# tencent-ailab/pika

Measured on NVIDIA H100. Metric: utterances/sec RNN-T train step (T=1000,U=150,V=6k), higher is better.
Workload: dtype bf16

## Files before the change

include/pika_b200.h:

```cpp
#ifndef PIKA_B200_H
#define PIKA_B200_H
#include <stdint.h>

#ifdef __cplusplus
extern "C" {
#endif

#define PK_F32 0
#define PK_BF16 1

const char* pk_last_error(void);
int pk_version(void);
long long pk_launch_count(void);

#define PK_GEMM_MAX_PAIRS 9
#define PK_SEL_ZERO 0
#define PK_SEL_ZB0 1
#define PK_SEL_ZB1 2
#define PK_SEL_KZ 3
#define PK_ACT_NONE 0
#define PK_ACT_RELU 1
#define PK_AUX_NONE 0
#define PK_AUX_ADD 1
#define PK_AUX_MASK_NZ 2

typedef struct {
    const void* ptr;
    int64_t dim[4];
    int64_t stride[3];
} pk_view4;

typedef struct {
    int n_pairs;
    pk_view4 a[PK_GEMM_MAX_PAIRS];
    pk_view4 b[PK_GEMM_MAX_PAIRS];
    int a_row_off[PK_GEMM_MAX_PAIRS];
    int b_row_off[PK_GEMM_MAX_PAIRS];
    int a_mn_major, b_mn_major;
    int a_sel2, a_sel3, b_sel2, b_sel3;
    int kz_count;
    pk_view4 c;
    int c_dtype;
    int c_accumulate;
    float alpha;
    const float* bias;
    int act;
    float drop_p;
    uint32_t drop_seed;
    int aux_mode;
    const void* aux;
    int aux_dtype;
    int64_t aux_stride[3];
    float aux_scale;
    int block_n;
    int k_splits;
    float* row_lse;
} pk_gemm_desc;

int pk_gemm_bf16(const pk_gemm_desc* desc, void* stream);
int pk_gemm_row_lse_parts(long long M, long long N, int block_n);

long long pk_rnnt_loss_workspace_bytes(int B, int T, int U1);
long long pk_rnnt_loss_colsum_workspace_bytes(int B, int T, int U1, int ldv);
int pk_rnnt_loss_fwd_bwd(const void* logits, int dtype, const int* labels, const int* frame_lens,
                         const int* label_lens, int B, int T, int U1, int V, int ldv, int ld_labels,
                         const float* grad_scale, float* costs, void* dlogits, float* dlogits_colsum, void* workspace,
                         long long workspace_bytes, void* stream);
int pk_rnnt_loss_fwd_bwd_lse(const void* logits, int dtype, const int* labels, const int* frame_lens,
                             const int* label_lens, int B, int T, int U1, int V, int ldv, int ld_labels,
                             const float* grad_scale, float* costs, void* dlogits, float* dlogits_colsum, void* workspace,
                             long long workspace_bytes, const float* row_lse, int n_parts, void* stream);

int pk_cast_split(const void* src, int src_dtype, long long ld_src, void* hi, void* lo, long long ld_dst,
                  long long rows, int cols, int cols_pad, float scale, void* stream);
int pk_attention_lse_stride(int T);
int pk_attention_fwd(const void* q, const void* k, const void* v, long long ld_qkv, void* out, long long ld_out, float* lse,
                     int B, int T, int heads, int dh, float alpha, float drop_p, uint32_t seed, void* stream);
int pk_attention_bwd(const void* q, const void* k, const void* v, long long ld_qkv, const void* out, long long ld_out,
                     const void* dout, long long ld_dout, const float* lse, float* dsum_ws, void* dq, void* dk, void* dv,
                     long long ld_dqkv, int B, int T, int heads, int dh, float alpha, float drop_p, uint32_t seed, void* stream);
long long pk_colstats_ws_floats(int C);
int pk_bn_fwd(const void* x, void* y, int dtype, long long rows, int C, const float* w, const float* b, float eps,
              int train, float momentum, float* run_mean, float* run_var, float* mean, float* rstd, float* stats_ws,
              void* stream);
int pk_bn_bwd(const void* dy, const void* x, void* dx, int dtype, long long rows, int C, const float* w,
              const float* mean, const float* rstd, int train, int relu_mask, float* dw, float* db, float* ws ,
              void* stream);
int pk_colsum(const void* x, int dtype, long long rows, int C, float* out, float* ws, void* stream);
int pk_layernorm_fwd(const void* x, void* y, int dtype, long long rows, int C, const float* w, const float* b, float eps,
                     float* mean, float* rstd, void* stream);
int pk_layernorm_bwd(const void* dy, const void* x, void* dx, int dtype, long long rows, int C, const float* w,
                     const float* mean, const float* rstd, float* dw, float* db, void* stream);
int pk_softmax_fwd(const float* S, long long ld_s, void* P, void* Pd, int dtype, long long ld_p, long long rows, int n,
                   float drop_p, uint32_t seed, void* stream);
int pk_softmax_masked_fwd(const float* S, long long ld_s, void* P, void* Pd, int dtype, long long ld_p, long long rows, int n,
                          int q_len, int heads, int causal, const uint8_t* key_pad, float drop_p, uint32_t seed, void* stream);
int pk_softmax_bwd(const float* dPd, long long ld_d, const void* P, long long ld_p, void* dS, int dtype, long long rows,
                   int n, float drop_p, uint32_t seed, void* stream);
#define PK_RELPOS_MAX 1024
int pk_softmax_masked_relpos_fwd(const float* S, long long ld_s, const float* QR, long long ld_r, void* P, void* Pd, int dtype,
                                 long long ld_p, long long rows, int n, int q_len, int heads, int causal, const uint8_t* key_pad,
                                 int max_rel, float* Pb, float drop_p, uint32_t seed, void* stream);
int pk_softmax_relpos_bwd(const float* dPd, long long ld_d, const float* G, long long ld_r, const void* P, long long ld_p, void* dS,
                          int dtype, long long rows, int n, int q_len, int heads, int max_rel, float* dSb, float drop_p,
                          uint32_t seed, void* stream);
int pk_dropout(const void* x, void* y, int dtype, long long n, float p, uint32_t seed, void* stream);
int pk_mask_nz(const void* dy, const void* y, void* dx, int dtype, long long n, float scale, void* stream);
int pk_add(const void* a, const void* b, void* o, int dtype, long long n, void* stream);
int pk_log_softmax(const void* x, int dtype, long long ld, float* y, long long rows, int n, float scale, void* stream);
int pk_joint_gate_fwd(const void* ex, const void* py, void* h, int dtype, int B, int T, int U1, int H, int ld_h, void* stream);
int pk_joint_gate_bwd(const void* ex, const void* py, const void* dh, void* dex, void* dpy, int dtype, int B, int T, int U1,
                      int H, void* stream);
int pk_lstm_cell_fwd(const float* gx, long long ld_gx, const float* gh, long long ld_gh, const float* c_prev, float* c_out,
                     void* h_out, int dtype, long long ld_h, float* gates_save, int B, int H, void* stream);
int pk_lstm_cell_bwd(const void* dh_out, long long ld_dho, const float* dh_rec, const float* dc_next, const float* gates,
                     const float* c, const float* c_prev, void* dgates, int dtype, float* dc_prev, int B, int H, void* stream);
int pk_embedding_fwd(const long long* idx, const float* table, int E, void* out, int dtype, int ld_out, long long n, void* stream);
int pk_embedding_bwd(const long long* idx, const void* dout, int dtype, int ld, int E, float* dtable, long long n,
                     long long padding_idx, void* stream);

int pk_absmax(const float* x, long long n, float* out, int* nan_flag, void* stream);
int pk_sgd_nesterov_clip(float* p, const float* g, float* buf, long long n, float lr, float momentum, float max_norm,
                         const float* absmax, const int* nan_flag, int first, void* stream);
int pk_bmuf_delta(const float* glob, const float* local, float* delta, long long n, void* stream);
int pk_bmuf_update(float* glob, float* local, float* delta_prev, const float* delta_sum, long long n, int world,
                   float block_momentum, float block_lr, void* stream);

long long pk_frontend_workspace_bytes(int B, int n_max, int t_max, int n_mel, int D);
int pk_frontend_fwd(const short* pcm, long long ld_pcm, const int* n_samples, const float* rate, const int* new_len,
                    const float* target_db, const int* n_frames, int B, int n_max, int t_max, int n_mel, int lctx,
                    int rctx, const float* window, const float* twiddle, const float* mel_w, const int* mel_lo,
                    const int* mel_hi, float preemph, int cmn, const float* offset, const float* scale, int f0, int fs,
                    int t0, int ts, void* out, int out_dtype, short* wave_i16_out, void* workspace,
                    long long workspace_bytes, int* err_flag, float dither, unsigned int dither_seed, void* stream);
int pk_fbank(const float* wave, long long ld_wave, const int* n_frames, int B, int t_max, int n_mel, const float* window,
             const float* twiddle, const float* mel_w, const int* mel_lo, const int* mel_hi, float preemph, float* feats,
             float dither, unsigned int dither_seed, void* stream);

int pk_beam_prepare(const int* next_ys, const int* step_ctx, int* t_idx, const void* enc, int dtype, int Tenc, int H, void* enc_hid,
                    const float* embed, int E, void* x_emb, int ld_x, int K, int blk, int rows, void* stream);
int pk_beam_lstm_cell(const float* gates, const int* next_ys, const int* step_ctx, int blk, void* h, int dtype, float* c, int rows, int H,
                      void* stream);
int pk_beam_step_end(int* step_ctx, const int* not_done, int max_steps, void* stream);
int pk_beam_gate(const float* a, void* h, int dtype, int rows, int H, void* stream);
int pk_row_lse(const void* x, int dtype, long long ld, float* lse, long long rows, int n, float scale, void* stream);
int pk_beam_advance(const float* logits, int ldv, const float* row_lse, float sm_scale, const int* t_idx, const int* num_frames, const int* max_len, float* scores,
                    int* next_ys, int* prev_ks, int* hyp_tok, int* hyp_len, float* fin_score, int* fin_step, int* fin_k,
                    int* fin_count, int* eos_top, int* done, int* not_done_total, int B, int K, int V, int L, int cap,
                    const int* step_ctx, int blk, int n_best, int beam_prune, void* stream);
int pk_beam_reorder(const int* prev_ks, const int* step_ctx, const void* h_in, const float* c_in, const int* t_in, void* h_out, float* c_out,
                    int* t_out, int dtype, int K, int H, int layers, int rows, void* stream);
typedef struct {
    const int* arc_off;
    const int* arc_ilabel;
    const double* arc_weight;
    const int* arc_next;
    const double* finals;
    int backoff_id, n_disambig;
    int disambig_ids[4];
} pk_lm_fst;
int pk_beam_advance_lm(const float* logits, int ldv, const float* row_lse, float sm_scale, const int* t_idx, const int* num_frames, const int* max_len, float* scores,
                       int* next_ys, int* prev_ks, int* hyp_tok, int* hyp_len, float* fin_score, int* fin_step, int* fin_k,
                       int* fin_count, int* eos_top, int* done, int* not_done_total, int B, int K, int V, int L, int cap,
                       const int* step_ctx, int blk, int n_best, int beam_prune, const pk_lm_fst* fst, double lm_scale, double nonblk_reward,
                       int* set_state, double* set_cost, int* set_n, float* lm_scores, int max_states, int* err_flag, void* stream);

typedef struct {
    const int* next_ys;
    const int* step_ctx;
    const int* hyp_tok;
    const int* hyp_len;
    int* slot;
    void* pool;
    long long n_entries;
    int blk, rows, S1, layers, D, dtype, init;
} pk_beam_xf_state;
int pk_beam_xf_taps(const pk_beam_xf_state* st, int layer, const float* embed, int E, const void* x_cur, void* taps, int ldc, void* stream);
int pk_beam_xf_attn(const pk_beam_xf_state* st, int layer, const void* qkv, int heads, const float* rel, int max_rel, void* out, void* stream);
int pk_beam_xf_select(const pk_beam_xf_state* st, const void* x, void* h, int H, void* stream);
int pk_beam_xf_slots(const pk_beam_xf_state* st, const int* prev_ks, int K, void* stream);

long long pk_lstm_seq_workspace_bytes(int H);
int pk_lstm_seq_fwd_ex(const float* gx, const void* w_hh_bf16, void* out, int out_dtype, int ldo, float* gates_save, float* cs,
                       const int* lens, int B, int U, int H, int n_dir, int reverse, void* ws, void* stream);
int pk_lstm_seq_bwd_ex(const void* dout, int dtype, int ldo, const float* gates_save, const float* cs, const void* w_hh_bf16,
                       void* dG_bf16, const int* lens, int B, int U, int H, int n_dir, int reverse, void* ws, void* stream);

int pk_gather_rows(const void* src, const int* idx, void* dst, int dtype, long long rows, int C, void* stream);
int pk_scatter_add_rows(const void* src, const int* idx, float* dst, int dtype, long long rows, int C, void* stream);
int pk_ce_grad(const void* z, int dtype, long long ld, const int* tok, const float* coef, float scale, void* dz,
               long long rows, int n, void* stream);

#ifdef __cplusplus
}
#endif
#endif
```

pika_b200/_lib.py:

```python
import ctypes
import os

_HERE = os.path.dirname(os.path.abspath(__file__))
LIB_PATH = os.path.join(_HERE, "libpika_b200.so")

PK_F32, PK_BF16 = 0, 1
SEL_ZERO, SEL_ZB0, SEL_ZB1, SEL_KZ = 0, 1, 2, 3
ACT_NONE, ACT_RELU = 0, 1
AUX_NONE, AUX_ADD, AUX_MASK_NZ = 0, 1, 2
MAX_PAIRS = 9


class PikaError(RuntimeError):
    pass


class View4(ctypes.Structure):
    _fields_ = [("ptr", ctypes.c_void_p), ("dim", ctypes.c_int64 * 4), ("stride", ctypes.c_int64 * 3)]


class GemmDesc(ctypes.Structure):
    _fields_ = [
        ("n_pairs", ctypes.c_int),
        ("a", View4 * MAX_PAIRS),
        ("b", View4 * MAX_PAIRS),
        ("a_row_off", ctypes.c_int * MAX_PAIRS),
        ("b_row_off", ctypes.c_int * MAX_PAIRS),
        ("a_mn_major", ctypes.c_int), ("b_mn_major", ctypes.c_int),
        ("a_sel2", ctypes.c_int), ("a_sel3", ctypes.c_int), ("b_sel2", ctypes.c_int), ("b_sel3", ctypes.c_int),
        ("kz_count", ctypes.c_int),
        ("c", View4),
        ("c_dtype", ctypes.c_int),
        ("c_accumulate", ctypes.c_int),
        ("alpha", ctypes.c_float),
        ("bias", ctypes.c_void_p),
        ("act", ctypes.c_int),
        ("drop_p", ctypes.c_float),
        ("drop_seed", ctypes.c_uint32),
        ("aux_mode", ctypes.c_int),
        ("aux", ctypes.c_void_p),
        ("aux_dtype", ctypes.c_int),
        ("aux_stride", ctypes.c_int64 * 3),
        ("aux_scale", ctypes.c_float),
        ("block_n", ctypes.c_int),
        ("k_splits", ctypes.c_int),
        ("row_lse", ctypes.c_void_p),
    ]


if not os.path.exists(LIB_PATH):
    raise ImportError(
        "pika_b200: %s is missing -- build it with `python -c 'import __graft_entry__ as g; g.build()'` "
        "(there is no CPU fallback)" % LIB_PATH)

lib = ctypes.CDLL(LIB_PATH)
lib.pk_last_error.restype = ctypes.c_char_p
lib.pk_launch_count.restype = ctypes.c_longlong
lib.pk_rnnt_loss_workspace_bytes.restype = ctypes.c_longlong

_vp, _i, _ll, _f, _u32 = ctypes.c_void_p, ctypes.c_int, ctypes.c_longlong, ctypes.c_float, ctypes.c_uint32


def _sig(name, argtypes, restype=ctypes.c_int):
    fn = getattr(lib, name)
    fn.argtypes = argtypes
    fn.restype = restype
    return fn


_sig("pk_gemm_bf16", [ctypes.POINTER(GemmDesc), _vp])
_sig("pk_gemm_row_lse_parts", [_ll, _ll, _i])
_sig("pk_rnnt_loss_workspace_bytes", [_i, _i, _i], ctypes.c_longlong)
_sig("pk_rnnt_loss_colsum_workspace_bytes", [_i, _i, _i, _i], ctypes.c_longlong)
_sig("pk_rnnt_loss_fwd_bwd", [_vp, _i, _vp, _vp, _vp, _i, _i, _i, _i, _i, _i, _vp, _vp, _vp, _vp, _vp, _ll, _vp])
_sig("pk_rnnt_loss_fwd_bwd_lse", [_vp, _i, _vp, _vp, _vp, _i, _i, _i, _i, _i, _i, _vp, _vp, _vp, _vp, _vp, _ll, _vp, _i, _vp])


def check(rc, what=""):
    if rc != 0:
        raise PikaError("%s failed (rc=%d): %s" % (what, rc, lib.pk_last_error().decode()))


def launch_count():
    return int(lib.pk_launch_count())
```

pika_b200/csrc/attention_tc.cu:

```cuda
#include <cstdlib>
#include <cstring>

#include "../../include/pika_b200.h"
#include "common.cuh"

namespace pk {
void count_launch();

constexpr int TA_BR = 128;
constexpr int TA_BC = 64;
constexpr int TA_NST = 4;
constexpr int TA_THREADS = 384;
constexpr float TA_LOG2E = 1.4426950408889634f;
constexpr float TA_LN2 = 0.6931471805599453f;

constexpr int TA_TILE_S = TA_BR * 128;
constexpr int TA_TILE_X = TA_BC * 128;
constexpr int TA_OFF_STAT = 0;
constexpr int TA_OFF_RING = 2 * TA_TILE_S;
constexpr int TA_OFF_VEC = TA_OFF_RING + TA_NST * 2 * TA_TILE_X;
constexpr int TA_OFF_BAR = TA_OFF_VEC + TA_NST * 2 * TA_BC * 4;
constexpr int TA_SMEM = TA_OFF_BAR + 256 + 1024;

struct AttnTcParams {
    CUtensorMap q, k, v, dout;
    __nv_bfloat16* out; long long ld_o;
    __nv_bfloat16* dq; __nv_bfloat16* dk; __nv_bfloat16* dv; long long ld_dqkv;
    float* lse;
    float* dsum;
    int B, T, heads, Tpad, Tp2;
    float alpha;
    uint32_t thresh16; float drop_scale; uint32_t seed;
};

PK_DEVICE void frag_a(const float (&x)[32], int kk, uint32_t (&a)[4]) {
    a[0] = pack_bf16x2(x[8 * kk + 0], x[8 * kk + 1]);
    a[1] = pack_bf16x2(x[8 * kk + 2], x[8 * kk + 3]);
    a[2] = pack_bf16x2(x[8 * kk + 4], x[8 * kk + 5]);
    a[3] = pack_bf16x2(x[8 * kk + 6], x[8 * kk + 7]);
}
PK_DEVICE float quad_max(float v) { return fmaxf(v, fmaxf(__shfl_xor_sync(0xffffffffu, v, 1), __shfl_xor_sync(0xffffffffu, fmaxf(v, __shfl_xor_sync(0xffffffffu, v, 1)), 2))); }
PK_DEVICE float quad_sum(float v) { v += __shfl_xor_sync(0xffffffffu, v, 1); return v + __shfl_xor_sync(0xffffffffu, v, 2); }

PK_DEVICE void store_tile(const float (&x)[32], __nv_bfloat16* base, long long ld, int row0, int T, int r0, int cq, float sc) {
#pragma unroll
    for (int h = 0; h < 2; ++h) {
        const int row = row0 + r0 + 8 * h;
        if (row >= T) continue;
        __nv_bfloat16* orow = base + (long long)row * ld;
#pragma unroll
        for (int nb = 0; nb < 8; ++nb)
            *reinterpret_cast<uint32_t*>(orow + nb * 8 + cq) = pack_bf16x2(x[nb * 4 + 2 * h] * sc, x[nb * 4 + 2 * h + 1] * sc);
    }
}

template <int MODE>
__global__ void __launch_bounds__(TA_THREADS, 1) attention_tc_kernel(const __grid_constant__ AttnTcParams p) {
    extern __shared__ uint8_t smem_raw[];
    uint8_t* smem = reinterpret_cast<uint8_t*>((reinterpret_cast<uintptr_t>(smem_raw) + 1023) & ~uintptr_t(1023));
    uint64_t* bars = reinterpret_cast<uint64_t*>(smem + TA_OFF_BAR);
    uint64_t* stat_full = bars;
    uint64_t* full_bar = bars + 1;
    uint64_t* empty_bar = full_bar + TA_NST;
    float* vec = reinterpret_cast<float*>(smem + TA_OFF_VEC);

    const int warp = threadIdx.x >> 5, lane = threadIdx.x & 31;
    const int T = p.T;
    const int bh = blockIdx.y, b = bh / p.heads, h = bh - b * p.heads;
    const int row_base = blockIdx.x * TA_BR;
    const int n_tiles = (T + TA_BC - 1) / TA_BC;

    if (threadIdx.x == 0) {
        tma_prefetch_desc(&p.q); tma_prefetch_desc(&p.k); tma_prefetch_desc(&p.v);
        if (MODE != 0) tma_prefetch_desc(&p.dout);
        mbar_init(stat_full, 1);
        for (int s = 0; s < TA_NST; ++s) { mbar_init(&full_bar[s], 1); mbar_init(&empty_bar[s], 2); }
        mbar_fence_init();
    }
    __syncthreads();

    if (warp < 4) {
        setmaxnreg_dec<40>();
        if (warp != 0) return;
        const uint32_t lead = elect_one_u32();
        const CUtensorMap* ma0 = (MODE == 2) ? &p.k : &p.q;
        const CUtensorMap* ma1 = (MODE == 2) ? &p.v : &p.dout;
        const CUtensorMap* mx1 = (MODE == 2) ? &p.q : &p.k;
        const CUtensorMap* mx2 = (MODE == 2) ? &p.dout : &p.v;
        mbar_arrive_expect_tx_p(stat_full, (MODE == 0 ? 1 : 2) * TA_TILE_S, lead);
        for (int half = 0; half < 2; ++half) {
            tma_load_3d_p(smem + TA_OFF_STAT + half * TA_TILE_X, ma0, stat_full, h * 64, row_base + half * 64, b, lead);
            if (MODE != 0) tma_load_3d_p(smem + TA_OFF_STAT + TA_TILE_S + half * TA_TILE_X, ma1, stat_full, h * 64, row_base + half * 64, b, lead);
        }
        int stage = 0;
        uint32_t phase = 0;
        for (int j = 0; j < n_tiles; ++j) {
            mbar_wait(&empty_bar[stage], phase ^ 1);
            uint8_t* x1 = smem + TA_OFF_RING + stage * 2 * TA_TILE_X;
            mbar_arrive_expect_tx_p(&full_bar[stage], 2 * TA_TILE_X + (MODE == 2 ? 2 * TA_BC * 4 : 0), lead);
            tma_load_3d_p(x1, mx1, &full_bar[stage], h * 64, j * TA_BC, b, lead);
            tma_load_3d_p(x1 + TA_TILE_X, mx2, &full_bar[stage], h * 64, j * TA_BC, b, lead);
            if (MODE == 2) {
                const size_t off = (size_t)bh * p.Tpad + (size_t)j * TA_BC;
                bulk_load_p(vec + (stage * 2 + 0) * TA_BC, p.lse + off, TA_BC * 4, &full_bar[stage], lead);
                bulk_load_p(vec + (stage * 2 + 1) * TA_BC, p.dsum + off, TA_BC * 4, &full_bar[stage], lead);
            }
            if (++stage == TA_NST) { stage = 0; phase ^= 1; }
        }
        return;
    }

    setmaxnreg_inc<232>();
    const int wg = (threadIdx.x >> 7) - 1;
    const int et = threadIdx.x & 127;
    const int r0 = (et >> 5) * 16 + (lane >> 2);
    const int cq = (lane & 3) * 2;
    const int srow0 = row_base + wg * 64;
    const uint64_t stat_row0 = (uint64_t)bh * (uint64_t)T;
    const float c2 = p.alpha * TA_LOG2E;
    const bool use_drop = p.thresh16 != 0u;
    const uint32_t sbase = smem_u32(smem);
    const uint64_t kdesc = make_smem_desc_sw128(0, 16, 1024);
    const uint64_t mdesc = make_smem_desc_sw128(0, 8192, 1024);
    auto kmaj = [&](uint32_t addr, int k4) { return kdesc + (uint64_t)((addr >> 4) & 0x3FFF) + (uint64_t)(k4 * 2); };
    auto mnmaj = [&](uint32_t addr, int k4) { return mdesc + (uint64_t)((addr >> 4) & 0x3FFF) + (uint64_t)(k4 * 128); };
    const uint32_t st0 = sbase + TA_OFF_STAT + wg * TA_TILE_X, st1 = st0 + TA_TILE_S;
    uint32_t row_salt[2];
    float lse2[2] = {0.f, 0.f}, dsum_r[2] = {0.f, 0.f};
#pragma unroll
    for (int hh = 0; hh < 2; ++hh) {
        const int srow = srow0 + r0 + 8 * hh;
        row_salt[hh] = drop_row_salt(stat_row0 + (uint64_t)srow, p.seed);
        if (MODE == 1 && srow < T) {
            lse2[hh] = p.lse[(size_t)bh * p.Tpad + srow] * TA_LOG2E;
            dsum_r[hh] = p.dsum[(size_t)bh * p.Tpad + srow];
        }
    }

    float acc0[32], acc1[32];
#pragma unroll
    for (int c = 0; c < 32; ++c) { acc0[c] = 0.f; acc1[c] = 0.f; }
    float m_run[2] = {-INFINITY, -INFINITY}, l_run[2] = {0.f, 0.f};

    mbar_wait(stat_full, 0);
    int stage = 0;
    uint32_t phase = 0;
    for (int j = 0; j < n_tiles; ++j) {
        const int col0 = j * TA_BC;
        const int nvalid = min(TA_BC, T - col0);
        mbar_wait(&full_bar[stage], phase);
        const uint32_t x1 = sbase + TA_OFF_RING + stage * 2 * TA_TILE_X, x2 = x1 + TA_TILE_X;
        float s[32], dp[32];
        wgmma_fence_acc(s);
        wgmma_fence();
#pragma unroll
        for (int k4 = 0; k4 < 4; ++k4) wgmma_ss_n64<0, 0>(s, kmaj(st0, k4), kmaj(x1, k4), k4 > 0 ? 1u : 0u);
        if (MODE != 0) {
            wgmma_fence_acc(dp);
#pragma unroll
            for (int k4 = 0; k4 < 4; ++k4) wgmma_ss_n64<0, 0>(dp, kmaj(st1, k4), kmaj(x2, k4), k4 > 0 ? 1u : 0u);
        }
        wgmma_commit();
        wgmma_wait<0>();
        wgmma_fence_acc(s);
        if (MODE != 0) wgmma_fence_acc(dp);
        if (nvalid < TA_BC) {
#pragma unroll
            for (int c = 0; c < 32; ++c) if ((c >> 2) * 8 + cq + (c & 1) >= nvalid) s[c] = -INFINITY;
        }
        if (MODE == 0) {
#pragma unroll
            for (int hh = 0; hh < 2; ++hh) {
                float mx = -INFINITY;
#pragma unroll
                for (int nb = 0; nb < 8; ++nb) mx = fmaxf(mx, fmaxf(s[nb * 4 + 2 * hh], s[nb * 4 + 2 * hh + 1]));
                const float m_new = fmaxf(m_run[hh], quad_max(mx) * c2);
                const float corr = ex2_approx(m_run[hh] - m_new);
#pragma unroll
                for (int nb = 0; nb < 8; ++nb) { acc0[nb * 4 + 2 * hh] *= corr; acc0[nb * 4 + 2 * hh + 1] *= corr; }
                float sum = 0.f;
#pragma unroll
                for (int nb = 0; nb < 8; ++nb) {
                    float* pr = &s[nb * 4 + 2 * hh];
                    pr[0] = ex2_approx(fmaf(pr[0], c2, -m_new));
                    pr[1] = ex2_approx(fmaf(pr[1], c2, -m_new));
                    sum += pr[0] + pr[1];
                    if (use_drop) {
                        const uint32_t km = drop_pair(row_salt[hh], (uint32_t)((col0 + nb * 8 + cq) >> 1), p.thresh16);
                        if (!(km & 1u)) pr[0] = 0.f;
                        if (!(km & 2u)) pr[1] = 0.f;
                    }
                }
                l_run[hh] = l_run[hh] * corr + sum;
                m_run[hh] = m_new;
            }
            wgmma_fence_acc(acc0);
            wgmma_fence();
#pragma unroll
            for (int kk = 0; kk < 4; ++kk) {
                uint32_t a[4];
                frag_a(s, kk, a);
                wgmma_rs_n64<1>(acc0, a, mnmaj(x2, kk), 1u);
            }
        } else {
            float pd[32], ds[32];
            const float* lse_t = vec + (stage * 2 + 0) * TA_BC;
            const float* dsum_t = lse_t + TA_BC;
            uint32_t qsalt[16];
            if (MODE == 2 && use_drop) {
#pragma unroll
                for (int c = 0; c < 16; ++c) qsalt[c] = drop_row_salt(stat_row0 + (uint64_t)(col0 + (c >> 1) * 8 + cq + (c & 1)), p.seed);
            }
#pragma unroll
            for (int hh = 0; hh < 2; ++hh) {
#pragma unroll
                for (int nb = 0; nb < 8; ++nb) {
                    uint32_t keep = 3u;
                    if (use_drop) {
                        if (MODE == 1) {
                            keep = drop_pair(row_salt[hh], (uint32_t)((col0 + nb * 8 + cq) >> 1), p.thresh16);
                        } else {
                            const uint32_t key = (uint32_t)(srow0 + r0 + 8 * hh);
                            const uint32_t bit = (key & 1u) ? 2u : 1u;
                            keep = ((drop_pair(qsalt[2 * nb], key >> 1, p.thresh16) & bit) ? 1u : 0u) |
                                   ((drop_pair(qsalt[2 * nb + 1], key >> 1, p.thresh16) & bit) ? 2u : 0u);
                        }
                    }
#pragma unroll
                    for (int e = 0; e < 2; ++e) {
                        const int c = nb * 4 + 2 * hh + e;
                        const int cl = nb * 8 + cq + e;
                        const float l2 = (MODE == 1) ? lse2[hh] : lse_t[cl] * TA_LOG2E;
                        const float dd = (MODE == 1) ? dsum_r[hh] : dsum_t[cl];
                        const float pr = ex2_approx(fmaf(s[c], c2, -l2));
                        const bool kp = (keep >> e) & 1u;
                        const float dpe = kp ? dp[c] * p.drop_scale : 0.f;
                        ds[c] = pr * (dpe - dd);
                        if (MODE == 2) pd[c] = kp ? pr * p.drop_scale : 0.f;
                    }
                }
            }
            wgmma_fence_acc(acc0);
            if (MODE == 2) wgmma_fence_acc(acc1);
            wgmma_fence();
#pragma unroll
            for (int kk = 0; kk < 4; ++kk) {
                uint32_t a[4];
                frag_a(ds, kk, a);
                if (MODE == 1) wgmma_rs_n64<1>(acc0, a, mnmaj(x1, kk), 1u);
                else wgmma_rs_n64<1>(acc0, a, mnmaj(x1, kk), 1u);
                if (MODE == 2) {
                    uint32_t a2[4];
                    frag_a(pd, kk, a2);
                    wgmma_rs_n64<1>(acc1, a2, mnmaj(x2, kk), 1u);
                }
            }
        }
        wgmma_commit();
        wgmma_wait<0>();
        wgmma_fence_acc(acc0);
        if (MODE == 2) wgmma_fence_acc(acc1);
        if (et == 0) mbar_arrive(&empty_bar[stage]);
        if (++stage == TA_NST) { stage = 0; phase ^= 1; }
    }

    if (MODE == 0) {
        float inv[2];
#pragma unroll
        for (int hh = 0; hh < 2; ++hh) {
            const float l = quad_sum(l_run[hh]);
            inv[hh] = p.drop_scale / l;
            const int srow = srow0 + r0 + 8 * hh;
            if ((lane & 3) == 0 && srow < p.Tpad) p.lse[(size_t)bh * p.Tpad + srow] = (m_run[hh] + log2f(l)) * TA_LN2;
        }
#pragma unroll
        for (int c = 0; c < 32; ++c) acc0[c] *= inv[(c >> 1) & 1];
        store_tile(acc0, p.out + (long long)b * T * p.ld_o + h * 64, p.ld_o, srow0, T, r0, cq, 1.f);
    } else if (MODE == 1) {
        store_tile(acc0, p.dq + (long long)b * T * p.ld_dqkv + h * 64, p.ld_dqkv, srow0, T, r0, cq, p.alpha);
    } else {
        store_tile(acc0, p.dk + (long long)b * T * p.ld_dqkv + h * 64, p.ld_dqkv, srow0, T, r0, cq, p.alpha);
        store_tile(acc1, p.dv + (long long)b * T * p.ld_dqkv + h * 64, p.ld_dqkv, srow0, T, r0, cq, 1.f);
    }
}

__global__ void __launch_bounds__(256) attention_rowdot_tc_kernel(const __nv_bfloat16* __restrict__ o, long long ld_o,
                                                                  const __nv_bfloat16* __restrict__ dout, long long ld_do, float* __restrict__ dsum,
                                                                  int B, int T, int heads, int Tpad) {
    const int lane = threadIdx.x & 31;
    const long long n = (long long)B * T * heads;
    for (long long w = (long long)blockIdx.x * 8 + (threadIdx.x >> 5); w < n; w += (long long)gridDim.x * 8) {
        const int h = (int)(w % heads);
        const long long bt = w / heads;
        const int tt = (int)(bt % T);
        const int b = (int)(bt / T);
        const uint32_t ov = *reinterpret_cast<const uint32_t*>(o + bt * ld_o + h * 64 + lane * 2);
        const uint32_t dv = *reinterpret_cast<const uint32_t*>(dout + bt * ld_do + h * 64 + lane * 2);
        const float s = warp_sum(bf16lo(ov) * bf16lo(dv) + bf16hi(ov) * bf16hi(dv));
        if (lane == 0) dsum[((long long)b * heads + h) * Tpad + tt] = s;
    }
    const long long npad = (long long)B * heads * (Tpad - T);
    for (long long i = (long long)blockIdx.x * blockDim.x + threadIdx.x; i < npad; i += (long long)gridDim.x * blockDim.x)
        dsum[(i / (Tpad - T)) * Tpad + T + i % (Tpad - T)] = 0.f;
}

static int attn_maps(AttnTcParams& p, const void* q, const void* k, const void* v, long long ld_qkv, const void* dout, long long ld_dout) {
    const unsigned long long dims[3] = {(unsigned long long)p.heads * 64, (unsigned long long)p.T, (unsigned long long)p.B};
    const unsigned box[3] = {64, TA_BC, 1};
    const unsigned long long st_qkv[2] = {(unsigned long long)ld_qkv * 2, (unsigned long long)ld_qkv * 2 * p.T};
    int rc;
    if ((rc = encode_tiled_bf16_3d(&p.q, q, dims, st_qkv, box, "attention q"))) return rc;
    if ((rc = encode_tiled_bf16_3d(&p.k, k, dims, st_qkv, box, "attention k"))) return rc;
    if ((rc = encode_tiled_bf16_3d(&p.v, v, dims, st_qkv, box, "attention v"))) return rc;
    if (dout) {
        const unsigned long long st_do[2] = {(unsigned long long)ld_dout * 2, (unsigned long long)ld_dout * 2 * p.T};
        if ((rc = encode_tiled_bf16_3d(&p.dout, dout, dims, st_do, box, "attention dout"))) return rc;
    }
    return 0;
}

template <int MODE> static int launch_attn(const AttnTcParams& p, cudaStream_t st) {
    auto kern = attention_tc_kernel<MODE>;
    static bool configured = false;
    if (!configured) {
        PK_CHECK_CUDA(cudaFuncSetAttribute(kern, cudaFuncAttributeMaxDynamicSharedMemorySize, TA_SMEM));
        configured = true;
    }
    dim3 grid((p.T + TA_BR - 1) / TA_BR, p.B * p.heads);
    kern<<<grid, TA_THREADS, TA_SMEM, st>>>(p);
    PK_CHECK_LAUNCH(); count_launch();
    return 0;
}

}

#define STREAM(s) reinterpret_cast<cudaStream_t>(s)

extern "C" int pk_attention_lse_stride(int T) { return (T + 63) / 64 * 64; }

#define ATTN_CHECKS()                                                                                                      \
    PK_CHECK_ARG(B > 0 && T > 0 && heads > 0, "bad dims");                                                                 \
    PK_CHECK_ARG(dh == 64, "fused attention supports head dim 64");                                                        \
    PK_CHECK_ARG(ld_qkv % 8 == 0 && ld_out % 8 == 0, "row strides must be multiples of 8 elements (16 bytes)");            \
    PK_CHECK_ARG(drop_p >= 0.f && drop_p < 1.f, "drop_p out of range");                                                    \
    PK_CHECK_ARG((long long)B * heads < 65536, "B * heads must be < 65536")

extern "C" int pk_attention_fwd(const void* q, const void* k, const void* v, long long ld_qkv, void* out, long long ld_out, float* lse,
                                int B, int T, int heads, int dh, float alpha, float drop_p, uint32_t seed, void* stream) {
    using namespace pk;
    ATTN_CHECKS();
    static thread_local AttnTcParams p;
    memset(&p, 0, sizeof(p));
    p.B = B; p.T = T; p.heads = heads; p.Tpad = pk_attention_lse_stride(T); p.Tp2 = (T + 1) / 2;
    int rc = attn_maps(p, q, k, v, ld_qkv, nullptr, 0);
    if (rc) return rc;
    p.out = (__nv_bfloat16*)out; p.ld_o = ld_out; p.lse = lse;
    p.alpha = alpha;
    p.thresh16 = drop_thresh16_of(drop_p); p.drop_scale = drop_scale16_of(p.thresh16); p.seed = seed;
    return launch_attn<0>(p, STREAM(stream));
}

extern "C" int pk_attention_bwd(const void* q, const void* k, const void* v, long long ld_qkv, const void* out, long long ld_out,
                                const void* dout, long long ld_dout, const float* lse, float* dsum_ws, void* dq, void* dk, void* dv,
                                long long ld_dqkv, int B, int T, int heads, int dh, float alpha, float drop_p, uint32_t seed, void* stream) {
    using namespace pk;
    ATTN_CHECKS();
    PK_CHECK_ARG(ld_dout % 8 == 0 && ld_dqkv % 8 == 0, "row strides must be multiples of 8 elements (16 bytes)");
    static thread_local AttnTcParams p;
    memset(&p, 0, sizeof(p));
    p.B = B; p.T = T; p.heads = heads; p.Tpad = pk_attention_lse_stride(T); p.Tp2 = (T + 1) / 2;
    int rc = attn_maps(p, q, k, v, ld_qkv, dout, ld_dout);
    if (rc) return rc;
    p.dq = (__nv_bfloat16*)dq; p.dk = (__nv_bfloat16*)dk; p.dv = (__nv_bfloat16*)dv; p.ld_dqkv = ld_dqkv;
    p.lse = const_cast<float*>(lse); p.dsum = dsum_ws;
    p.alpha = alpha;
    p.thresh16 = drop_thresh16_of(drop_p); p.drop_scale = drop_scale16_of(p.thresh16); p.seed = seed;
    const long long n = (long long)B * T * heads;
    const long long rmax = (long long)num_sms() * 16;
    const int rgrid = (int)((n + 7) / 8 < rmax ? (n + 7) / 8 : rmax);
    attention_rowdot_tc_kernel<<<rgrid, 256, 0, STREAM(stream)>>>((const __nv_bfloat16*)out, ld_out, (const __nv_bfloat16*)dout, ld_dout, dsum_ws,
                                                                   B, T, heads, p.Tpad);
    PK_CHECK_LAUNCH(); count_launch();
    rc = launch_attn<1>(p, STREAM(stream));
    if (rc) return rc;
    return launch_attn<2>(p, STREAM(stream));
}
```

pika_b200/csrc/common.cuh:

```cuda
#pragma once
#include <cuda.h>
#include <cuda_bf16.h>
#include <cuda_runtime.h>
#include <stdint.h>

#define PK_DEVICE __device__ __forceinline__

namespace pk {

void set_last_error(const char* fmt, ...);
#define PK_CHECK_ARG(cond, msg)                                       \
    do {                                                              \
        if (!(cond)) {                                                \
            pk::set_last_error("%s:%d: %s", __FILE__, __LINE__, msg); \
            return -1;                                                \
        }                                                             \
    } while (0)
#define PK_CHECK_CUDA(expr)                                                                     \
    do {                                                                                        \
        cudaError_t e__ = (expr);                                                               \
        if (e__ != cudaSuccess) {                                                               \
            pk::set_last_error("%s:%d: CUDA error %s", __FILE__, __LINE__, cudaGetErrorString(e__)); \
            return -2;                                                                          \
        }                                                                                       \
    } while (0)
#define PK_CHECK_LAUNCH() PK_CHECK_CUDA(cudaGetLastError())

int num_sms();
int encode_tiled_bf16_3d(CUtensorMap* out, const void* ptr, const unsigned long long (&dims)[3], const unsigned long long (&strides_bytes)[2],
                         const unsigned (&box)[3], const char* what);

enum DType : int { F32 = 0, BF16 = 1 };

template <typename T> PK_DEVICE float to_f32(T v);
template <> PK_DEVICE float to_f32<float>(float v) { return v; }
template <> PK_DEVICE float to_f32<__nv_bfloat16>(__nv_bfloat16 v) { return __bfloat162float(v); }
template <typename T> PK_DEVICE T from_f32(float v);
template <> PK_DEVICE float from_f32<float>(float v) { return v; }
template <> PK_DEVICE __nv_bfloat16 from_f32<__nv_bfloat16>(float v) { return __float2bfloat16_rn(v); }

PK_DEVICE uint32_t pack_bf16x2(float lo, float hi) {
    __nv_bfloat162 v = __floats2bfloat162_rn(lo, hi);
    return *reinterpret_cast<uint32_t*>(&v);
}
PK_DEVICE float ex2_approx(float x) {
    float y;
    asm("ex2.approx.ftz.f32 %0, %1;" : "=f"(y) : "f"(x));
    return y;
}
PK_DEVICE float bf16lo(uint32_t v) { return __uint_as_float(v << 16); }
PK_DEVICE float bf16hi(uint32_t v) { return __uint_as_float(v & 0xffff0000u); }

PK_DEVICE uint32_t hash_u32(uint64_t idx, uint32_t seed) {
    uint32_t x = (uint32_t)idx ^ (seed * 0x9E3779B9u);
    uint32_t y = (uint32_t)(idx >> 32) + seed;
    x ^= x >> 16; x *= 0x7feb352dU; x ^= x >> 15; x *= 0x846ca68bU; x ^= x >> 16;
    x += y * 0x85ebca6bU;
    x ^= x >> 13; x *= 0xc2b2ae35U; x ^= x >> 16;
    return x;
}
PK_DEVICE bool drop_keep(uint64_t idx, uint32_t seed, uint32_t thresh) { return hash_u32(idx, seed) >= thresh; }

PK_DEVICE uint32_t drop_row_salt(uint64_t grow, uint32_t seed) { return hash_u32(grow, seed); }
PK_DEVICE uint32_t drop_pair(uint32_t salt, uint32_t kp, uint32_t thresh16) {
    uint32_t x = (salt + kp) * 0x9E3779B1u;
    x ^= x >> 15; x *= 0x85EBCA77u; x ^= x >> 13;
    return ((x & 0xFFFFu) >= thresh16 ? 1u : 0u) | ((x >> 16) >= thresh16 ? 2u : 0u);
}
__host__ __device__ inline uint32_t drop_thresh16_of(float p) {
    if (p <= 0.f) return 0u;
    const double t = (double)p * 65536.0 + 0.5;
    const uint32_t r = t >= 65535.0 ? 65535u : (uint32_t)t;
    return r == 0 ? 1u : r;
}
__host__ __device__ inline float drop_scale16_of(uint32_t thresh16) { return thresh16 ? 1.f / (1.f - (float)thresh16 / 65536.f) : 1.f; }

PK_DEVICE float warp_sum(float v) {
#pragma unroll
    for (int o = 16; o > 0; o >>= 1) v += __shfl_xor_sync(0xffffffffu, v, o);
    return v;
}
PK_DEVICE float warp_max(float v) {
#pragma unroll
    for (int o = 16; o > 0; o >>= 1) v = fmaxf(v, __shfl_xor_sync(0xffffffffu, v, o));
    return v;
}

PK_DEVICE uint32_t smem_u32(const void* p) { return (uint32_t)__cvta_generic_to_shared(p); }

PK_DEVICE bool elect_one() {
    uint32_t pred;
    asm volatile(
        "{\n\t.reg .pred p;\n\t.reg .b32 r;\n\t"
        "elect.sync r|p, 0xffffffff;\n\t"
        "selp.u32 %0, 1, 0, p;\n\t}\n"
        : "=r"(pred));
    return pred != 0;
}

PK_DEVICE void mbar_init(uint64_t* bar, uint32_t count) {
    asm volatile("mbarrier.init.shared::cta.b64 [%0], %1;" ::"r"(smem_u32(bar)), "r"(count));
}
PK_DEVICE void mbar_fence_init() { asm volatile("fence.mbarrier_init.release.cluster;" ::: "memory"); }
PK_DEVICE void mbar_arrive_expect_tx(uint64_t* bar, uint32_t bytes) {
    asm volatile("mbarrier.arrive.expect_tx.shared::cta.b64 _, [%0], %1;" ::"r"(smem_u32(bar)), "r"(bytes)
                 : "memory");
}
PK_DEVICE void mbar_arrive(uint64_t* bar) {
    asm volatile("mbarrier.arrive.shared::cta.b64 _, [%0];" ::"r"(smem_u32(bar)) : "memory");
}
PK_DEVICE bool mbar_try_wait(uint64_t* bar, uint32_t parity) {
    uint32_t done;
    asm volatile(
        "{\n\t.reg .pred p;\n\t"
        "mbarrier.try_wait.parity.shared::cta.b64 p, [%1], %2;\n\t"
        "selp.u32 %0, 1, 0, p;\n\t}\n"
        : "=r"(done)
        : "r"(smem_u32(bar)), "r"(parity)
        : "memory");
    return done != 0;
}
PK_DEVICE void mbar_wait(uint64_t* bar, uint32_t parity) {
    while (!mbar_try_wait(bar, parity)) {
    }
}

PK_DEVICE void tma_prefetch_desc(const CUtensorMap* m) {
    asm volatile("prefetch.tensormap [%0];" ::"l"(reinterpret_cast<uint64_t>(m)) : "memory");
}
PK_DEVICE void tma_load_4d(void* smem_dst, const CUtensorMap* m, uint64_t* bar, int c0, int c1, int c2, int c3) {
    asm volatile(
        "cp.async.bulk.tensor.4d.shared::cluster.global.tile.mbarrier::complete_tx::bytes"
        " [%0], [%1, {%3, %4, %5, %6}], [%2];" ::"r"(smem_u32(smem_dst)),
        "l"(reinterpret_cast<uint64_t>(m)), "r"(smem_u32(bar)), "r"(c0), "r"(c1), "r"(c2), "r"(c3)
        : "memory");
}
PK_DEVICE void tma_load_3d(void* smem_dst, const CUtensorMap* m, uint64_t* bar, int c0, int c1, int c2) {
    asm volatile(
        "cp.async.bulk.tensor.3d.shared::cluster.global.tile.mbarrier::complete_tx::bytes"
        " [%0], [%1, {%3, %4, %5}], [%2];" ::"r"(smem_u32(smem_dst)),
        "l"(reinterpret_cast<uint64_t>(m)), "r"(smem_u32(bar)), "r"(c0), "r"(c1), "r"(c2)
        : "memory");
}
PK_DEVICE void bulk_load(void* smem_dst, const void* gsrc, uint32_t bytes, uint64_t* bar) {
    asm volatile("cp.async.bulk.shared::cluster.global.mbarrier::complete_tx::bytes [%0], [%1], %2, [%3];" ::"r"(smem_u32(smem_dst)),
                 "l"(reinterpret_cast<uint64_t>(gsrc)), "r"(bytes), "r"(smem_u32(bar))
                 : "memory");
}
PK_DEVICE void tma_store_4d(const CUtensorMap* m, const void* smem_src, int c0, int c1, int c2, int c3) {
    asm volatile(
        "cp.async.bulk.tensor.4d.global.shared::cta.tile.bulk_group [%0, {%2, %3, %4, %5}], [%1];" ::"l"(
            reinterpret_cast<uint64_t>(m)),
        "r"(smem_u32(smem_src)), "r"(c0), "r"(c1), "r"(c2), "r"(c3)
        : "memory");
}
PK_DEVICE void tma_reduce_add_4d(const CUtensorMap* m, const void* smem_src, int c0, int c1, int c2, int c3) {
    asm volatile(
        "cp.reduce.async.bulk.tensor.4d.global.shared::cta.add.tile.bulk_group [%0, {%2, %3, %4, %5}], [%1];" ::"l"(
            reinterpret_cast<uint64_t>(m)),
        "r"(smem_u32(smem_src)), "r"(c0), "r"(c1), "r"(c2), "r"(c3)
        : "memory");
}
constexpr uint64_t kL2EvictNormal = 0x1000000000000000ull;
constexpr uint64_t kL2EvictFirst = 0x12F0000000000000ull;
constexpr uint64_t kL2EvictLast = 0x14F0000000000000ull;
PK_DEVICE void tma_load_4d_hint(void* smem_dst, const CUtensorMap* m, uint64_t* bar, int c0, int c1, int c2, int c3, uint64_t pol) {
    asm volatile(
        "cp.async.bulk.tensor.4d.shared::cluster.global.tile.mbarrier::complete_tx::bytes.L2::cache_hint"
        " [%0], [%1, {%3, %4, %5, %6}], [%2], %7;" ::"r"(smem_u32(smem_dst)),
        "l"(reinterpret_cast<uint64_t>(m)), "r"(smem_u32(bar)), "r"(c0), "r"(c1), "r"(c2), "r"(c3), "l"(pol)
        : "memory");
}
PK_DEVICE void tma_store_4d_hint(const CUtensorMap* m, const void* smem_src, int c0, int c1, int c2, int c3, uint64_t pol) {
    asm volatile(
        "cp.async.bulk.tensor.4d.global.shared::cta.tile.bulk_group.L2::cache_hint [%0, {%2, %3, %4, %5}], [%1], %6;" ::"l"(
            reinterpret_cast<uint64_t>(m)),
        "r"(smem_u32(smem_src)), "r"(c0), "r"(c1), "r"(c2), "r"(c3), "l"(pol)
        : "memory");
}
PK_DEVICE void tma_store_commit() { asm volatile("cp.async.bulk.commit_group;" ::: "memory"); }
template <int N> PK_DEVICE void tma_store_wait_read() {
    asm volatile("cp.async.bulk.wait_group.read %0;" ::"n"(N) : "memory");
}
template <int N> PK_DEVICE void tma_store_wait() { asm volatile("cp.async.bulk.wait_group %0;" ::"n"(N) : "memory"); }
PK_DEVICE void fence_proxy_async_smem() { asm volatile("fence.proxy.async.shared::cta;" ::: "memory"); }

PK_DEVICE uint64_t make_smem_desc_sw128(uint32_t smem_addr, uint32_t lbo_bytes, uint32_t sbo_bytes) {
    uint64_t d = 0;
    d |= (uint64_t)((smem_addr >> 4) & 0x3FFF);
    d |= (uint64_t)((lbo_bytes >> 4) & 0x3FFF) << 16;
    d |= (uint64_t)((sbo_bytes >> 4) & 0x3FFF) << 32;
    d |= (uint64_t)1 << 62;
    return d;
}
PK_DEVICE void wgmma_fence() { asm volatile("wgmma.fence.sync.aligned;" ::: "memory"); }
PK_DEVICE void wgmma_commit() { asm volatile("wgmma.commit_group.sync.aligned;" ::: "memory"); }
template <int N> PK_DEVICE void wgmma_wait() { asm volatile("wgmma.wait_group.sync.aligned %0;" ::"n"(N) : "memory"); }
template <int R> PK_DEVICE void wgmma_fence_acc(float (&d)[R]) {
#pragma unroll
    for (int i = 0; i < R; ++i) asm volatile("" : "+f"(d[i])::"memory");
}
template <int N> PK_DEVICE void setmaxnreg_inc() { asm volatile("setmaxnreg.inc.sync.aligned.u32 %0;" ::"n"(N)); }
template <int N> PK_DEVICE void setmaxnreg_dec() { asm volatile("setmaxnreg.dec.sync.aligned.u32 %0;" ::"n"(N)); }

template <int TA, int TB> PK_DEVICE void wgmma_ss_n64(float (&d)[32], uint64_t a, uint64_t b, uint32_t acc) {
    asm volatile(
        "{\n\t.reg .pred p;\n\tsetp.ne.b32 p, %34, 0;\n\t"
        "wgmma.mma_async.sync.aligned.m64n64k16.f32.bf16.bf16 {%0, %1, %2, %3, %4, %5, %6, %7, %8, %9, %10, %11, %12, %13, %14, %15, %16, %17, %18, %19, %20, %21, %22, %23, %24, %25, %26, %27, %28, %29, %30, %31}, %32, %33, p, 1, 1, %35, %36;\n\t}\n"
        : "+f"(d[0]), "+f"(d[1]), "+f"(d[2]), "+f"(d[3]), "+f"(d[4]), "+f"(d[5]), "+f"(d[6]), "+f"(d[7]), "+f"(d[8]), "+f"(d[9]), "+f"(d[10]), "+f"(d[11]), "+f"(d[12]), "+f"(d[13]), "+f"(d[14]), "+f"(d[15]), "+f"(d[16]), "+f"(d[17]), "+f"(d[18]), "+f"(d[19]), "+f"(d[20]), "+f"(d[21]), "+f"(d[22]), "+f"(d[23]), "+f"(d[24]), "+f"(d[25]), "+f"(d[26]), "+f"(d[27]), "+f"(d[28]), "+f"(d[29]), "+f"(d[30]), "+f"(d[31])
        : "l"(a), "l"(b), "r"(acc), "n"(TA), "n"(TB));
}
template <int TB> PK_DEVICE void wgmma_rs_n64(float (&d)[32], const uint32_t (&a)[4], uint64_t b, uint32_t acc) {
    asm volatile(
        "{\n\t.reg .pred p;\n\tsetp.ne.b32 p, %37, 0;\n\t"
        "wgmma.mma_async.sync.aligned.m64n64k16.f32.bf16.bf16 {%0, %1, %2, %3, %4, %5, %6, %7, %8, %9, %10, %11, %12, %13, %14, %15, %16, %17, %18, %19, %20, %21, %22, %23, %24, %25, %26, %27, %28, %29, %30, %31}, {%32, %33, %34, %35}, %36, p, 1, 1, %38;\n\t}\n"
        : "+f"(d[0]), "+f"(d[1]), "+f"(d[2]), "+f"(d[3]), "+f"(d[4]), "+f"(d[5]), "+f"(d[6]), "+f"(d[7]), "+f"(d[8]), "+f"(d[9]), "+f"(d[10]), "+f"(d[11]), "+f"(d[12]), "+f"(d[13]), "+f"(d[14]), "+f"(d[15]), "+f"(d[16]), "+f"(d[17]), "+f"(d[18]), "+f"(d[19]), "+f"(d[20]), "+f"(d[21]), "+f"(d[22]), "+f"(d[23]), "+f"(d[24]), "+f"(d[25]), "+f"(d[26]), "+f"(d[27]), "+f"(d[28]), "+f"(d[29]), "+f"(d[30]), "+f"(d[31])
        : "r"(a[0]), "r"(a[1]), "r"(a[2]), "r"(a[3]), "l"(b), "r"(acc), "n"(TB));
}
template <int TA, int TB> PK_DEVICE void wgmma_ss_n128(float (&d)[64], uint64_t a, uint64_t b, uint32_t acc) {
    asm volatile(
        "{\n\t.reg .pred p;\n\tsetp.ne.b32 p, %66, 0;\n\t"
        "wgmma.mma_async.sync.aligned.m64n128k16.f32.bf16.bf16 {%0, %1, %2, %3, %4, %5, %6, %7, %8, %9, %10, %11, %12, %13, %14, %15, %16, %17, %18, %19, %20, %21, %22, %23, %24, %25, %26, %27, %28, %29, %30, %31, %32, %33, %34, %35, %36, %37, %38, %39, %40, %41, %42, %43, %44, %45, %46, %47, %48, %49, %50, %51, %52, %53, %54, %55, %56, %57, %58, %59, %60, %61, %62, %63}, %64, %65, p, 1, 1, %67, %68;\n\t}\n"
        : "+f"(d[0]), "+f"(d[1]), "+f"(d[2]), "+f"(d[3]), "+f"(d[4]), "+f"(d[5]), "+f"(d[6]), "+f"(d[7]), "+f"(d[8]), "+f"(d[9]), "+f"(d[10]), "+f"(d[11]), "+f"(d[12]), "+f"(d[13]), "+f"(d[14]), "+f"(d[15]), "+f"(d[16]), "+f"(d[17]), "+f"(d[18]), "+f"(d[19]), "+f"(d[20]), "+f"(d[21]), "+f"(d[22]), "+f"(d[23]), "+f"(d[24]), "+f"(d[25]), "+f"(d[26]), "+f"(d[27]), "+f"(d[28]), "+f"(d[29]), "+f"(d[30]), "+f"(d[31]), "+f"(d[32]), "+f"(d[33]), "+f"(d[34]), "+f"(d[35]), "+f"(d[36]), "+f"(d[37]), "+f"(d[38]), "+f"(d[39]), "+f"(d[40]), "+f"(d[41]), "+f"(d[42]), "+f"(d[43]), "+f"(d[44]), "+f"(d[45]), "+f"(d[46]), "+f"(d[47]), "+f"(d[48]), "+f"(d[49]), "+f"(d[50]), "+f"(d[51]), "+f"(d[52]), "+f"(d[53]), "+f"(d[54]), "+f"(d[55]), "+f"(d[56]), "+f"(d[57]), "+f"(d[58]), "+f"(d[59]), "+f"(d[60]), "+f"(d[61]), "+f"(d[62]), "+f"(d[63])
        : "l"(a), "l"(b), "r"(acc), "n"(TA), "n"(TB));
}
template <int TA, int TB> PK_DEVICE void wgmma_ss_n256(float (&d)[128], uint64_t a, uint64_t b, uint32_t acc) {
    asm volatile(
        "{\n\t.reg .pred p;\n\tsetp.ne.b32 p, %130, 0;\n\t"
        "wgmma.mma_async.sync.aligned.m64n256k16.f32.bf16.bf16 {%0, %1, %2, %3, %4, %5, %6, %7, %8, %9, %10, %11, %12, %13, %14, %15, %16, %17, %18, %19, %20, %21, %22, %23, %24, %25, %26, %27, %28, %29, %30, %31, %32, %33, %34, %35, %36, %37, %38, %39, %40, %41, %42, %43, %44, %45, %46, %47, %48, %49, %50, %51, %52, %53, %54, %55, %56, %57, %58, %59, %60, %61, %62, %63, %64, %65, %66, %67, %68, %69, %70, %71, %72, %73, %74, %75, %76, %77, %78, %79, %80, %81, %82, %83, %84, %85, %86, %87, %88, %89, %90, %91, %92, %93, %94, %95, %96, %97, %98, %99, %100, %101, %102, %103, %104, %105, %106, %107, %108, %109, %110, %111, %112, %113, %114, %115, %116, %117, %118, %119, %120, %121, %122, %123, %124, %125, %126, %127}, %128, %129, p, 1, 1, %131, %132;\n\t}\n"
        : "+f"(d[0]), "+f"(d[1]), "+f"(d[2]), "+f"(d[3]), "+f"(d[4]), "+f"(d[5]), "+f"(d[6]), "+f"(d[7]), "+f"(d[8]), "+f"(d[9]), "+f"(d[10]), "+f"(d[11]), "+f"(d[12]), "+f"(d[13]), "+f"(d[14]), "+f"(d[15]), "+f"(d[16]), "+f"(d[17]), "+f"(d[18]), "+f"(d[19]), "+f"(d[20]), "+f"(d[21]), "+f"(d[22]), "+f"(d[23]), "+f"(d[24]), "+f"(d[25]), "+f"(d[26]), "+f"(d[27]), "+f"(d[28]), "+f"(d[29]), "+f"(d[30]), "+f"(d[31]), "+f"(d[32]), "+f"(d[33]), "+f"(d[34]), "+f"(d[35]), "+f"(d[36]), "+f"(d[37]), "+f"(d[38]), "+f"(d[39]), "+f"(d[40]), "+f"(d[41]), "+f"(d[42]), "+f"(d[43]), "+f"(d[44]), "+f"(d[45]), "+f"(d[46]), "+f"(d[47]), "+f"(d[48]), "+f"(d[49]), "+f"(d[50]), "+f"(d[51]), "+f"(d[52]), "+f"(d[53]), "+f"(d[54]), "+f"(d[55]), "+f"(d[56]), "+f"(d[57]), "+f"(d[58]), "+f"(d[59]), "+f"(d[60]), "+f"(d[61]), "+f"(d[62]), "+f"(d[63]), "+f"(d[64]), "+f"(d[65]), "+f"(d[66]), "+f"(d[67]), "+f"(d[68]), "+f"(d[69]), "+f"(d[70]), "+f"(d[71]), "+f"(d[72]), "+f"(d[73]), "+f"(d[74]), "+f"(d[75]), "+f"(d[76]), "+f"(d[77]), "+f"(d[78]), "+f"(d[79]), "+f"(d[80]), "+f"(d[81]), "+f"(d[82]), "+f"(d[83]), "+f"(d[84]), "+f"(d[85]), "+f"(d[86]), "+f"(d[87]), "+f"(d[88]), "+f"(d[89]), "+f"(d[90]), "+f"(d[91]), "+f"(d[92]), "+f"(d[93]), "+f"(d[94]), "+f"(d[95]), "+f"(d[96]), "+f"(d[97]), "+f"(d[98]), "+f"(d[99]), "+f"(d[100]), "+f"(d[101]), "+f"(d[102]), "+f"(d[103]), "+f"(d[104]), "+f"(d[105]), "+f"(d[106]), "+f"(d[107]), "+f"(d[108]), "+f"(d[109]), "+f"(d[110]), "+f"(d[111]), "+f"(d[112]), "+f"(d[113]), "+f"(d[114]), "+f"(d[115]), "+f"(d[116]), "+f"(d[117]), "+f"(d[118]), "+f"(d[119]), "+f"(d[120]), "+f"(d[121]), "+f"(d[122]), "+f"(d[123]), "+f"(d[124]), "+f"(d[125]), "+f"(d[126]), "+f"(d[127])
        : "l"(a), "l"(b), "r"(acc), "n"(TA), "n"(TB));
}

PK_DEVICE uint32_t cluster_ctarank() { uint32_t r; asm volatile("mov.u32 %0, %%cluster_ctarank;" : "=r"(r)); return r; }
PK_DEVICE uint32_t cluster_nctarank() { uint32_t r; asm volatile("mov.u32 %0, %%cluster_nctarank;" : "=r"(r)); return r; }
PK_DEVICE void cluster_sync_all() {
    asm volatile("barrier.cluster.arrive.release.aligned;" ::: "memory");
    asm volatile("barrier.cluster.wait.acquire.aligned;" ::: "memory");
}

PK_DEVICE uint32_t elect_one_u32() {
    uint32_t pred;
    asm volatile(
        "{\n\t.reg .pred p;\n\t.reg .b32 r;\n\t"
        "elect.sync r|p, 0xffffffff;\n\t"
        "selp.u32 %0, 1, 0, p;\n\t}\n"
        : "=r"(pred));
    return pred;
}
PK_DEVICE void mbar_arrive_expect_tx_p(uint64_t* bar, uint32_t bytes, uint32_t pred) {
    asm volatile("{\n\t.reg .pred q;\n\tsetp.ne.b32 q, %2, 0;\n\t@q mbarrier.arrive.expect_tx.shared::cta.b64 _, [%0], %1;\n\t}\n" ::"r"(smem_u32(bar)),
                 "r"(bytes), "r"(pred)
                 : "memory");
}
PK_DEVICE void tma_load_3d_p(void* smem_dst, const CUtensorMap* m, uint64_t* bar, int c0, int c1, int c2, uint32_t pred) {
    asm volatile(
        "{\n\t.reg .pred q;\n\tsetp.ne.b32 q, %6, 0;\n\t"
        "@q cp.async.bulk.tensor.3d.shared::cluster.global.tile.mbarrier::complete_tx::bytes [%0], [%1, {%3, %4, %5}], [%2];\n\t}\n" ::"r"(
            smem_u32(smem_dst)),
        "l"(reinterpret_cast<uint64_t>(m)), "r"(smem_u32(bar)), "r"(c0), "r"(c1), "r"(c2), "r"(pred)
        : "memory");
}
PK_DEVICE void bulk_load_p(void* smem_dst, const void* gsrc, uint32_t bytes, uint64_t* bar, uint32_t pred) {
    asm volatile(
        "{\n\t.reg .pred q;\n\tsetp.ne.b32 q, %4, 0;\n\t"
        "@q cp.async.bulk.shared::cluster.global.mbarrier::complete_tx::bytes [%0], [%1], %2, [%3];\n\t}\n" ::"r"(smem_u32(smem_dst)),
        "l"(reinterpret_cast<uint64_t>(gsrc)), "r"(bytes), "r"(smem_u32(bar)), "r"(pred)
        : "memory");
}
PK_DEVICE void tma_load_4d_hint_p(void* smem_dst, const CUtensorMap* m, uint64_t* bar, int c0, int c1, int c2, int c3, uint64_t pol, uint32_t pred) {
    asm volatile(
        "{\n\t.reg .pred q;\n\tsetp.ne.b32 q, %8, 0;\n\t"
        "@q cp.async.bulk.tensor.4d.shared::cluster.global.tile.mbarrier::complete_tx::bytes.L2::cache_hint"
        " [%0], [%1, {%3, %4, %5, %6}], [%2], %7;\n\t}\n" ::"r"(smem_u32(smem_dst)),
        "l"(reinterpret_cast<uint64_t>(m)), "r"(smem_u32(bar)), "r"(c0), "r"(c1), "r"(c2), "r"(c3), "l"(pol), "r"(pred)
        : "memory");
}
PK_DEVICE void tma_store_4d_hint_p(const CUtensorMap* m, const void* smem_src, int c0, int c1, int c2, int c3, uint64_t pol, uint32_t pred) {
    asm volatile(
        "{\n\t.reg .pred q;\n\tsetp.ne.b32 q, %7, 0;\n\t"
        "@q cp.async.bulk.tensor.4d.global.shared::cta.tile.bulk_group.L2::cache_hint [%0, {%2, %3, %4, %5}], [%1], %6;\n\t}\n" ::"l"(
            reinterpret_cast<uint64_t>(m)),
        "r"(smem_u32(smem_src)), "r"(c0), "r"(c1), "r"(c2), "r"(c3), "l"(pol), "r"(pred)
        : "memory");
}
PK_DEVICE void tma_reduce_add_4d_p(const CUtensorMap* m, const void* smem_src, int c0, int c1, int c2, int c3, uint32_t pred) {
    asm volatile(
        "{\n\t.reg .pred q;\n\tsetp.ne.b32 q, %6, 0;\n\t"
        "@q cp.reduce.async.bulk.tensor.4d.global.shared::cta.add.tile.bulk_group [%0, {%2, %3, %4, %5}], [%1];\n\t}\n" ::"l"(
            reinterpret_cast<uint64_t>(m)),
        "r"(smem_u32(smem_src)), "r"(c0), "r"(c1), "r"(c2), "r"(c3), "r"(pred)
        : "memory");
}
PK_DEVICE void tma_store_commit_p(uint32_t pred) {
    asm volatile("{\n\t.reg .pred q;\n\tsetp.ne.b32 q, %0, 0;\n\t@q cp.async.bulk.commit_group;\n\t}\n" ::"r"(pred) : "memory");
}
template <int N> PK_DEVICE void tma_store_wait_read_p(uint32_t pred) {
    asm volatile("{\n\t.reg .pred q;\n\tsetp.ne.b32 q, %1, 0;\n\t@q cp.async.bulk.wait_group.read %0;\n\t}\n" ::"n"(N), "r"(pred) : "memory");
}

PK_DEVICE void named_bar_sync(int id, int nthreads) { asm volatile("bar.sync %0, %1;" ::"r"(id), "r"(nthreads) : "memory"); }

PK_DEVICE void stmatrix_x4(uint32_t addr, uint32_t r0, uint32_t r1, uint32_t r2, uint32_t r3) {
    asm volatile("stmatrix.sync.aligned.m8n8.x4.shared.b16 [%0], {%1, %2, %3, %4};" ::"r"(addr), "r"(r0), "r"(r1), "r"(r2), "r"(r3)
                 : "memory");
}
PK_DEVICE uint4 lds_u32x4(uint32_t addr) {
    uint4 v;
    asm volatile("ld.shared.v4.u32 {%0, %1, %2, %3}, [%4];" : "=r"(v.x), "=r"(v.y), "=r"(v.z), "=r"(v.w) : "r"(addr) : "memory");
    return v;
}
PK_DEVICE float2 lds_f32x2(uint32_t addr) {
    float2 v;
    asm volatile("ld.shared.v2.f32 {%0, %1}, [%2];" : "=f"(v.x), "=f"(v.y) : "r"(addr) : "memory");
    return v;
}
PK_DEVICE void sts_f32(uint32_t addr, float v) { asm volatile("st.shared.f32 [%0], %1;" ::"r"(addr), "f"(v) : "memory"); }
PK_DEVICE uint32_t bf16x2_max(uint32_t a, uint32_t b) {
    uint32_t d;
    asm("max.bf16x2 %0, %1, %2;" : "=r"(d) : "r"(a), "r"(b));
    return d;
}

}
```

pika_b200/csrc/runtime.cu:

```cuda
#include <atomic>
#include <cstdarg>
#include <cstdio>

#include "../../include/pika_b200.h"
#include "common.cuh"

namespace pk {
static thread_local char g_err[512] = "";
static std::atomic<long long> g_launches{0};

void set_last_error(const char* fmt, ...) {
    va_list ap;
    va_start(ap, fmt);
    vsnprintf(g_err, sizeof(g_err), fmt, ap);
    va_end(ap);
}
void count_launch() { g_launches.fetch_add(1, std::memory_order_relaxed); }
int num_sms() {
    static int n = 0;
    if (n == 0) {
        int dev = 0;
        cudaGetDevice(&dev);
        cudaDeviceGetAttribute(&n, cudaDevAttrMultiProcessorCount, dev);
        if (n <= 0) n = 132;
    }
    return n;
}
}

extern "C" const char* pk_last_error(void) { return pk::g_err; }
extern "C" int pk_version(void) { return 102; }
extern "C" long long pk_launch_count(void) { return pk::g_launches.load(); }
```

pika_b200/engine.py:

```python
import math
import weakref

import torch

from . import kernels as K

_PRECISION = "bf16"
_WEIGHT_EPOCH = 0
_SEED = [0x5EED]
_DROPOUT_ENABLED = True


def set_precision(p):
    global _PRECISION
    assert p in ("bf16", "fp32")
    _PRECISION = p


def get_precision():
    return _PRECISION


def act_dtype():
    return torch.bfloat16 if _PRECISION == "bf16" else torch.float32


def invalidate_weights():
    global _WEIGHT_EPOCH
    _WEIGHT_EPOCH += 1


def set_seed(seed):
    _SEED[0] = seed & 0x7FFFFFFF


def set_dropout_enabled(flag):
    global _DROPOUT_ENABLED
    _DROPOUT_ENABLED = bool(flag)


def _next_seed():
    _SEED[0] = (_SEED[0] * 1103515245 + 12345) & 0x7FFFFFFF
    return _SEED[0]


def _drop(p, training):
    return float(p) if (training and _DROPOUT_ENABLED and p > 0) else 0.0


def stage_act(x):
    if x.dtype == torch.bfloat16:
        return [x]
    x2 = x.reshape(-1, x.shape[-1])
    hi = torch.empty(x2.shape, dtype=torch.bfloat16, device=x.device)
    lo = torch.empty_like(hi)
    K.cast_split(x2, hi, lo)
    return [hi.view(x.shape), lo.view(x.shape)]


_wcache = {}


def _prune_wcache():
    if len(_wcache) > 512:
        for k in [k for k, v in _wcache.items() if any(r() is None for r in v[2])]:
            del _wcache[k]


def _same_objects(refs, params):
    return len(refs) == len(params) and all(r() is p for r, p in zip(refs, params))


def stage_weight(params, cols_pad=None, scale=None):
    params = params if isinstance(params, (list, tuple)) else [params]
    key = (tuple(id(p) for p in params), _PRECISION, cols_pad)
    stamp = (tuple(p._version for p in params), _WEIGHT_EPOCH, tuple(p.data_ptr() for p in params))
    hit = _wcache.get(key)
    if hit is not None and hit[0] == stamp and _same_objects(hit[2], params):
        return hit[1]
    mats = [p.detach().reshape(p.shape[0], -1) for p in params]
    Kdim = mats[0].shape[1]
    kp = cols_pad or Kdim
    n = sum(m.shape[0] for m in mats)
    hi = torch.empty(n, kp, dtype=torch.bfloat16, device=mats[0].device)
    lo = torch.empty_like(hi) if _PRECISION == "fp32" else None
    r = 0
    for i, m in enumerate(mats):
        K.cast_split(m, hi[r:r + m.shape[0]], None if lo is None else lo[r:r + m.shape[0]], cols_pad=kp,
                     scale=1.0 if scale is None else scale[i])
        r += m.shape[0]
    parts = [hi] if lo is None else [hi, lo]
    _prune_wcache()
    _wcache[key] = (stamp, parts, tuple(weakref.ref(p) for p in params))
    return parts


def stage_conv1d_weight(weight, ld):
    key = (id(weight), _PRECISION, "conv1d", ld)
    stamp = (weight._version, _WEIGHT_EPOCH, weight.data_ptr())
    hit = _wcache.get(key)
    if hit is not None and hit[0] == stamp and _same_objects(hit[2], [weight]):
        return hit[1]
    N, C, Kw = weight.shape
    mat = torch.zeros(N, Kw, ld, dtype=torch.float32, device=weight.device)
    mat[:, :, :C] = weight.detach().permute(0, 2, 1)
    mat = mat.view(N, Kw * ld)
    hi = torch.empty(N, Kw * ld, dtype=torch.bfloat16, device=weight.device)
    lo = torch.empty_like(hi) if _PRECISION == "fp32" else None
    K.cast_split(mat, hi, lo)
    parts = [hi] if lo is None else [hi, lo]
    _prune_wcache()
    _wcache[key] = (stamp, parts, (weakref.ref(weight),))
    return parts


def _cat_bias(params):
    if len(params) == 1:
        return params[0].detach()
    key = (tuple(id(p) for p in params), "bias")
    stamp = (tuple(p._version for p in params), _WEIGHT_EPOCH, tuple(p.data_ptr() for p in params))
    hit = _wcache.get(key)
    if hit is not None and hit[0] == stamp and _same_objects(hit[2], params):
        return hit[1]
    out = torch.empty(sum(p.numel() for p in params), dtype=torch.float32, device=params[0].device)
    r = 0
    for p in params:
        out[r:r + p.numel()].copy_(p.detach())
        r += p.numel()
    _wcache[key] = (stamp, out, tuple(weakref.ref(p) for p in params))
    return out


def gemm_parts(a_taps, b_taps, c, **kw):
    A, Bm, aro, bro = [], [], [], []
    a_off = kw.pop("a_row_off", None)
    b_off = kw.pop("b_row_off", None)
    for t, (ap, bp) in enumerate(zip(a_taps, b_taps)):
        combos = [(0, 0)]
        if len(ap) > 1 and len(bp) > 1:
            combos += [(0, 1), (1, 0)]
        elif len(ap) > 1:
            combos += [(1, 0)]
        elif len(bp) > 1:
            combos += [(0, 1)]
        for (i, j) in combos:
            A.append(ap[i])
            Bm.append(bp[j])
            aro.append(a_off[t] if a_off else 0)
            bro.append(b_off[t] if b_off else 0)
    return K.gemm(A, Bm, c, a_row_off=aro, b_row_off=bro, **kw)


def grad_of(p):
    if p.grad is None:
        p.grad = torch.zeros_like(p, memory_format=torch.contiguous_format)
    return p.grad


def _new(shape, dtype=None, like=None, zero=False):
    dev = like.device if like is not None else "cuda"
    f = torch.zeros if zero else torch.empty
    return f(shape, dtype=dtype or act_dtype(), device=dev)


class LinearFn(torch.autograd.Function):

    @staticmethod
    def forward(ctx, x, residual, act, drop_p, seed, nw, premasked, mask_input_scale, *params):
        weights = list(params[:nw])
        biases = list(params[nw:]) if len(params) > nw else None
        M, Kd = x.shape
        w_parts = stage_weight(weights, cols_pad=x.shape[1] if x.shape[1] != weights[0].shape[1] else None)
        N = w_parts[0].shape[0]
        y = _new((M, N), like=x)
        bias = _cat_bias(biases) if biases is not None else None
        a_parts = stage_act(x)
        gemm_parts([a_parts], [w_parts], y, bias=bias, act=K.ACT_RELU if act else K.ACT_NONE, drop_p=drop_p,
                   drop_seed=seed, aux=residual, aux_mode=K.AUX_ADD if residual is not None else K.AUX_NONE)
        ctx.weights, ctx.biases, ctx.act, ctx.drop_p, ctx.seed = weights, biases, act, drop_p, seed
        ctx.premasked, ctx.mask_input_scale = premasked, mask_input_scale
        ctx.has_res = residual is not None
        ctx.save_for_backward(x, y if act else None)
        ctx.a_parts, ctx.w_parts = a_parts, w_parts
        return y

    @staticmethod
    def backward(ctx, dy):
        x, y = ctx.saved_tensors
        dy = dy.contiguous()
        M, N = dy.shape
        if ctx.premasked:
            dpre = dy
        elif ctx.act:
            dpre = torch.empty_like(dy)
            K.mask_nz(dy, y, dpre, 1.0 / (1.0 - ctx.drop_p) if ctx.drop_p > 0 else 1.0)
        elif ctx.drop_p > 0:
            dpre = torch.empty_like(dy)
            K.dropout(dy, dpre, ctx.drop_p, ctx.seed)
        else:
            dpre = dy
        d_parts = stage_act(dpre)
        dx = None
        if ctx.needs_input_grad[0]:
            dx = torch.empty_like(x)
            if ctx.mask_input_scale > 0:
                gemm_parts([d_parts], [ctx.w_parts], dx, b_mn=True, aux=x, aux_mode=K.AUX_MASK_NZ, aux_scale=ctx.mask_input_scale)
            else:
                gemm_parts([d_parts], [ctx.w_parts], dx, b_mn=True)
            if dx.shape[1] != x.shape[1]:
                dx = dx[:, :x.shape[1]]
        r = 0
        dbias = None
        if ctx.biases is not None:
            dbias = torch.empty(N, dtype=torch.float32, device=dy.device)
            K.colsum(dpre, dbias)
        for i, w in enumerate(ctx.weights):
            n_i = w.shape[0]
            g = grad_of(w).view(n_i, -1)
            gemm_parts([[p[:, r:r + n_i] for p in d_parts]], [[p[:, :g.shape[1]] for p in ctx.a_parts]], g, a_mn=True, b_mn=True)
            if ctx.biases is not None:
                grad_of(ctx.biases[i]).copy_(dbias[r:r + n_i])
            r += n_i
        n_par = len(ctx.weights) + (len(ctx.biases) if ctx.biases is not None else 0)
        return (dx, (dy if ctx.has_res else None), None, None, None, None, None, None) + (None,) * n_par


def linear(x, weights, biases=None, act=False, drop_p=0.0, residual=None, premasked=False, mask_input_scale=0.0):
    weights = list(weights) if isinstance(weights, (list, tuple)) else [weights]
    if biases is not None and not isinstance(biases, (list, tuple)):
        biases = [biases]
    params = weights + (list(biases) if biases is not None else [])
    if x.dtype != torch.bfloat16 or x.shape[1] % 8 != 0:
        mask_input_scale = 0.0
    return LinearFn.apply(x, residual, act, drop_p, _next_seed() if drop_p > 0 else 0, len(weights), premasked, mask_input_scale, *params)


class TdnnFn(torch.autograd.Function):

    @staticmethod
    def forward(ctx, x, weight, bias, dil, stride, premasked=False):
        B, T, C = x.shape
        ctx.premasked = premasked
        N = weight.shape[0]
        t_out = (T - 2 * dil - 1) // stride + 1
        w_parts = stage_weight(weight)
        a_parts = stage_act(x)
        span = (t_out - 1) * stride + 1
        a_taps = [[p[:, k * dil: k * dil + span: stride, :] for p in a_parts] for k in range(3)]
        b_taps = [[p[:, k * C:(k + 1) * C] for p in w_parts] for k in range(3)]
        y = _new((B, t_out, N), like=x)
        gemm_parts(a_taps, b_taps, y, a_sel=(K.SEL_ZB0, K.SEL_ZERO), b_sel=(K.SEL_ZERO, K.SEL_ZERO), bias=bias.detach(),
                   act=K.ACT_RELU)
        ctx.save_for_backward(x, y)
        ctx.a_parts, ctx.w_parts, ctx.weight, ctx.bias = a_parts, w_parts, weight, bias
        ctx.dil, ctx.stride, ctx.t_out = dil, stride, t_out
        return y

    @staticmethod
    def backward(ctx, dy):
        x, y = ctx.saved_tensors
        B, T, C = x.shape
        N = ctx.weight.shape[0]
        dil, stride, t_out = ctx.dil, ctx.stride, ctx.t_out
        if ctx.premasked:
            dpre = dy.contiguous()
        else:
            dpre = torch.empty_like(y)
            K.mask_nz(dy.contiguous(), y, dpre, 1.0)
        d_parts = stage_act(dpre)
        b_taps = [[p[:, k * C:(k + 1) * C] for p in ctx.w_parts] for k in range(3)]
        dx = None
        if ctx.needs_input_grad[0]:
            if stride == 1:
                dx = torch.empty_like(x)
                gemm_parts([d_parts] * 3, b_taps, dx, b_mn=True, a_sel=(K.SEL_ZB0, K.SEL_ZERO),
                           b_sel=(K.SEL_ZERO, K.SEL_ZERO), a_row_off=[0, -dil, -2 * dil])
            else:
                assert len({(k * dil) % stride for k in range(3)}) == 3, "overlapping strided taps not supported"
                dx = torch.zeros_like(x)
                span = (t_out - 1) * stride + 1
                for k in range(3):
                    gemm_parts([d_parts], [b_taps[k]], dx[:, k * dil: k * dil + span: stride, :], b_mn=True,
                               a_sel=(K.SEL_ZB0, K.SEL_ZERO), b_sel=(K.SEL_ZERO, K.SEL_ZERO))
        gw = grad_of(ctx.weight).view(N, 3 * C)
        span = (t_out - 1) * stride + 1
        for k in range(3):
            xt = [p[:, k * dil: k * dil + span: stride, :] for p in ctx.a_parts]
            gemm_parts([d_parts], [xt], gw[:, k * C:(k + 1) * C], a_mn=True, b_mn=True, a_sel=(K.SEL_KZ, K.SEL_ZERO),
                       b_sel=(K.SEL_KZ, K.SEL_ZERO), kz_count=B)
        K.colsum(dpre.view(B * t_out, N), grad_of(ctx.bias))
        return dx, None, None, None, None, None


class CausalConvFn(torch.autograd.Function):

    @staticmethod
    def forward(ctx, x, weight, bias):
        B, T, ld = x.shape
        N, C, Kw = weight.shape
        assert ld >= C and ld % 8 == 0
        xp = _new((B, T + Kw - 1, ld), like=x, zero=True)
        xp[:, Kw - 1:, :] = x
        a_parts = [p.as_strided((B, T, Kw * ld), ((T + Kw - 1) * ld, ld, 1)) for p in stage_act(xp)]
        w_parts = stage_conv1d_weight(weight, ld)
        y = _new((B, T, N), like=x)
        gemm_parts([a_parts], [w_parts], y, a_sel=(K.SEL_ZB0, K.SEL_ZERO), b_sel=(K.SEL_ZERO, K.SEL_ZERO), bias=bias.detach(),
                   act=K.ACT_RELU)
        ctx.save_for_backward(y)
        ctx.a_parts, ctx.w_parts, ctx.weight, ctx.bias, ctx.shape = a_parts, w_parts, weight, bias, (B, T, ld, N, C, Kw)
        return y

    @staticmethod
    def backward(ctx, dy):
        (y,) = ctx.saved_tensors
        B, T, ld, N, C, Kw = ctx.shape
        dpre = torch.empty_like(y)
        K.mask_nz(dy.contiguous(), y, dpre, 1.0)
        d_parts = stage_act(dpre)
        dx = None
        if ctx.needs_input_grad[0]:
            per = 3 if len(d_parts) > 1 else Kw
            dx = _new((B, T, ld), dtype=torch.float32 if len(d_parts) > 1 else None, like=y)
            for k0 in range(0, Kw, per):
                ks = list(range(k0, min(Kw, k0 + per)))
                b_taps = [[p[:, k * ld:(k + 1) * ld] for p in ctx.w_parts] for k in ks]
                gemm_parts([d_parts] * len(ks), b_taps, dx, b_mn=True, a_sel=(K.SEL_ZB0, K.SEL_ZERO), b_sel=(K.SEL_ZERO, K.SEL_ZERO),
                           a_row_off=[Kw - 1 - k for k in ks], accumulate=k0 > 0)
        gw = torch.empty(N, Kw * ld, dtype=torch.float32, device=y.device)
        gemm_parts([d_parts], [ctx.a_parts], gw, a_mn=True, b_mn=True, a_sel=(K.SEL_KZ, K.SEL_ZERO), b_sel=(K.SEL_KZ, K.SEL_ZERO),
                   kz_count=B)
        grad_of(ctx.weight).copy_(gw.view(N, Kw, ld)[:, :, :C].permute(0, 2, 1))
        K.colsum(dpre.view(B * T, N), grad_of(ctx.bias))
        return dx, None, None


class BatchNormFn(torch.autograd.Function):
    @staticmethod
    def forward(ctx, x, bn, train, _w=None, _b=None, relu_input=False):
        ctx.relu_input = relu_input
        rows, C = x.shape
        y = torch.empty_like(x)
        mean = torch.empty(C, dtype=torch.float32, device=x.device)
        rstd = torch.empty_like(mean)
        ws = torch.empty(2 * C, dtype=torch.float32, device=x.device)
        K.bn_fwd(x, y, bn.weight.detach(), bn.bias.detach(), bn.eps, train, bn.momentum if bn.momentum is not None else 0.1,
                 bn.running_mean, bn.running_var, mean, rstd, ws)
        if train and bn.num_batches_tracked is not None:
            bn.num_batches_tracked += 1
        ctx.save_for_backward(x, mean, rstd)
        ctx.bn, ctx.train = bn, train
        return y

    @staticmethod
    def backward(ctx, dy):
        x, mean, rstd = ctx.saved_tensors
        dx = torch.empty_like(x)
        K.bn_bwd(dy.contiguous(), x, dx, ctx.bn.weight.detach(), mean, rstd, ctx.train, ctx.relu_input, grad_of(ctx.bn.weight),
                 grad_of(ctx.bn.bias))
        return dx, None, None, None, None, None


class LayerNormFn(torch.autograd.Function):
    @staticmethod
    def forward(ctx, x, ln, _w=None, _b=None):
        rows, C = x.shape
        y = torch.empty_like(x)
        mean = torch.empty(rows, dtype=torch.float32, device=x.device)
        rstd = torch.empty_like(mean)
        K.layernorm_fwd(x, y, ln.weight.detach(), ln.bias.detach(), ln.eps, mean, rstd)
        ctx.save_for_backward(x, mean, rstd)
        ctx.ln = ln
        return y

    @staticmethod
    def backward(ctx, dy):
        x, mean, rstd = ctx.saved_tensors
        dx = torch.empty_like(x)
        K.layernorm_bwd(dy.contiguous(), x, dx, ctx.ln.weight.detach(), mean, rstd, grad_of(ctx.ln.weight), grad_of(ctx.ln.bias))
        return dx, None, None, None


_FUSED_ATTN = True


class AttentionFn(torch.autograd.Function):

    @staticmethod
    def forward(ctx, qkv, heads, drop_p, seed, causal=False, key_pad=None, rel=None):
        B, T, D3 = qkv.shape
        D = D3 // 3
        dh = D // heads
        masked = causal or key_pad is not None
        ctx.rel = rel
        ctx.fused = _FUSED_ATTN and qkv.dtype == torch.bfloat16 and dh == 64 and not masked and rel is None
        if ctx.fused:
            qkv = qkv.contiguous()
            out = _new((B, T, D), like=qkv)
            lse = torch.zeros(B * heads * K.attention_lse_stride(T), dtype=torch.float32, device=qkv.device)
            alpha = 1.0 / math.sqrt(dh)
            K.attention_fwd(qkv, out, lse, heads, alpha, drop_p, seed)
            ctx.save_for_backward(qkv, out, lse)
            ctx.meta = (B, T, D, heads, dh, 0, drop_p, seed, alpha)
            return out
        Tp = (T + 7) // 8 * 8
        parts = stage_act(qkv)

        def head_view(p, which):
            return p[:, :, which * D:(which + 1) * D].view(B, T, heads, dh).permute(0, 2, 1, 3)

        q, k, v = ([head_view(p, i) for p in parts] for i in range(3))
        S = torch.empty(B, heads, T, Tp, dtype=torch.float32, device=qkv.device)
        alpha = 1.0 / math.sqrt(dh)
        gemm_parts([q], [k], S[:, :, :, :T], alpha=alpha)
        P = _new((B, heads, T, Tp), like=qkv)
        Pd = _new((B, heads, T, Tp), like=qkv) if drop_p > 0 else P
        rel_out = {}
        if rel is not None:
            nb = rel.shape[0]
            r_parts = stage_weight(rel)
            qc = [torch.empty(B * T, D, dtype=torch.bfloat16, device=qkv.device) for _ in parts]
            K.cast_split(qkv.view(B * T, D3)[:, :D], qc[0], qc[1] if len(qc) > 1 else None, scale=alpha)
            qc = [p.view(B * T * heads, dh) for p in qc]
            QR = torch.empty(B * T * heads, (nb + 7) // 8 * 8, dtype=torch.float32, device=qkv.device)
            gemm_parts([qc], [r_parts], QR[:, :nb])
            Pb = torch.empty_like(QR)
            K.softmax_masked_relpos_fwd(S, QR, P, Pd, Pb, T, heads, causal, key_pad, nb // 2, drop_p, seed)
            del QR
            pb_parts = [p[:, :nb] for p in stage_act(Pb)]
            Y = torch.empty(B * T * heads, dh, dtype=torch.float32, device=qkv.device)
            gemm_parts([pb_parts], [r_parts], Y, b_mn=True)
            rel_out = dict(aux=Y.view(B, T, heads, dh).permute(0, 2, 1, 3), aux_mode=K.AUX_ADD)
            ctx.r_parts, ctx.qc, ctx.pb_parts = r_parts, qc, pb_parts
        elif masked:
            K.softmax_masked_fwd(S, P, Pd, T, T, heads, causal, key_pad, drop_p, seed)
        else:
            K.softmax_fwd(S, P, Pd, T, drop_p, seed)
        del S
        out = _new((B, T, D), like=qkv)
        pd_parts = stage_act(Pd)
        gemm_parts([[p[:, :, :, :T] for p in pd_parts]], [v], out.view(B, T, heads, dh).permute(0, 2, 1, 3), b_mn=True, **rel_out)
        ctx.save_for_backward(qkv, P)
        ctx.pd_parts, ctx.parts = pd_parts, parts
        ctx.meta = (B, T, D, heads, dh, Tp, drop_p, seed, alpha)
        return out

    @staticmethod
    def backward(ctx, dout):
        if ctx.fused:
            qkv, out, lse = ctx.saved_tensors
            B, T, D, heads, dh, _, drop_p, seed, alpha = ctx.meta
            dqkv = torch.empty_like(qkv)
            K.attention_bwd(qkv, out, dout.contiguous(), lse, dqkv, heads, alpha, drop_p, seed)
            return dqkv, None, None, None, None, None, None
        qkv, P = ctx.saved_tensors
        B, T, D, heads, dh, Tp, drop_p, seed, alpha = ctx.meta
        dout = dout.contiguous()

        def head_view(p, which, d=D):
            return p[:, :, which * d:(which + 1) * d].view(B, T, heads, dh).permute(0, 2, 1, 3)

        q, k, v = ([head_view(p, i) for p in ctx.parts] for i in range(3))
        do_parts = stage_act(dout)
        do = [p.view(B, T, heads, dh).permute(0, 2, 1, 3) for p in do_parts]
        dqkv = torch.empty_like(qkv)
        gemm_parts([[p[:, :, :, :T] for p in ctx.pd_parts]], [do], head_view(dqkv, 2), a_mn=True, b_mn=True)
        dPd = torch.empty(B, heads, T, Tp, dtype=torch.float32, device=qkv.device)
        gemm_parts([do], [v], dPd[:, :, :, :T])
        dS = torch.empty_like(P)
        rel, rel_dq = ctx.rel, {}
        if rel is not None:
            nb = rel.shape[0]
            do2 = [p.view(B * T * heads, dh) for p in do_parts]
            G = torch.empty(B * T * heads, (nb + 7) // 8 * 8, dtype=torch.float32, device=qkv.device)
            gemm_parts([do2], [ctx.r_parts], G[:, :nb])
            dSb = torch.empty_like(G)
            K.softmax_relpos_bwd(dPd, G, P, dS, dSb, T, heads, nb // 2, drop_p, seed)
            del G
            dsb_parts = [p[:, :nb] for p in stage_act(dSb)]
            Z = torch.empty(B * T * heads, dh, dtype=torch.float32, device=qkv.device)
            gemm_parts([dsb_parts], [ctx.r_parts], Z, b_mn=True, alpha=alpha)
            rel_dq = dict(aux=Z.view(B, T, heads, dh).permute(0, 2, 1, 3), aux_mode=K.AUX_ADD)
            gemm_parts([dsb_parts, ctx.pb_parts], [ctx.qc, do2], grad_of(rel), a_mn=True, b_mn=True)
        else:
            K.softmax_bwd(dPd, P, dS, T, drop_p, seed)
        del dPd
        ds_parts = [p[:, :, :, :T] for p in stage_act(dS)]
        gemm_parts([ds_parts], [k], head_view(dqkv, 0), b_mn=True, alpha=alpha, **rel_dq)
        gemm_parts([ds_parts], [q], head_view(dqkv, 1), a_mn=True, b_mn=True, alpha=alpha)
        return dqkv, None, None, None, None, None, None


class EmbeddingFn(torch.autograd.Function):
    @staticmethod
    def forward(ctx, idx, emb, ld, _w=None):
        n = idx.numel()
        out = _new((n, ld), like=emb.weight)
        K.embedding_fwd(idx.reshape(-1).contiguous(), emb.weight.detach(), out)
        ctx.idx, ctx.emb = idx.reshape(-1).contiguous(), emb
        return out

    @staticmethod
    def backward(ctx, dout):
        K.embedding_bwd(ctx.idx, dout.contiguous(), grad_of(ctx.emb.weight), ctx.emb.padding_idx)
        return None, None, None, None


def _lstm_step_maps(lens, B, U, rev):
    r = torch.arange(U, dtype=torch.int32, device=lens.device).view(U, 1)
    b = torch.arange(B, dtype=torch.int32, device=lens.device).view(1, B)
    L = lens.view(1, B).clamp(0, U)
    other = (L - 1 - r) if rev else r.expand(U, B)
    live = r < L
    src = b * U + torch.where(live, other, torch.zeros_like(other))
    dsrc = torch.where(live, b * U + other, torch.full_like(other, B * U))
    to_time = torch.where(live, other * B + b, torch.full_like(other, U * B))
    return src, dsrc, to_time


class LstmLayerFn(torch.autograd.Function):

    @staticmethod
    def forward(ctx, x, lens, *params):
        B, U, E = x.shape
        n_dir = len(params) // 4
        dirs = [params[4 * d:4 * d + 4] for d in range(n_dir)]
        H = dirs[0][1].shape[1]
        G4 = 4 * H
        wih_parts = [stage_weight(p[0], cols_pad=E if E != p[0].shape[1] else None) for p in dirs]
        whh_parts = stage_weight([p[1] for p in dirs])
        x_parts = stage_act(x)
        gx = torch.empty(n_dir, B, U, G4, dtype=torch.float32, device=x.device)
        for d, (w_ih, w_hh, b_ih, b_hh) in enumerate(dirs):
            bsum = torch.empty(G4, dtype=torch.float32, device=x.device)
            K.add(b_ih.detach(), b_hh.detach(), bsum)
            gemm_parts([[p.view(B * U, E) for p in x_parts]], [wih_parts[d]], gx[d].view(B * U, G4), bias=bsum)
        out = _new((B, U, n_dir * H), like=x)
        gates = torch.empty(n_dir, U, B, G4, dtype=torch.float32, device=x.device)
        cs = torch.empty(n_dir, U, B, H, dtype=torch.float32, device=x.device)
        ctx.persistent = (x.dtype == torch.bfloat16 and H % 64 == 0 and
                          n_dir * H // 8 <= torch.cuda.get_device_properties(x.device).multi_processor_count)
        if ctx.persistent:
            K.lstm_seq_fwd_ex(gx, whh_parts[0], out, gates, cs, lens)
        else:
            for d in range(n_dir):
                whh = [p[d * G4:(d + 1) * G4] for p in whh_parts]
                out_d = out[:, :, d * H:(d + 1) * H]
                if lens is None and d == 0:
                    gx_s, h_s = (lambda t: gx[d][:, t, :]), (lambda t: out_d[:, t, :])
                else:
                    src, _, _ = _lstm_step_maps(lens if lens is not None else _full_lens(B, U, x.device), B, U, d == 1)
                    gxs = torch.empty(U * B, G4, dtype=torch.float32, device=x.device)
                    K.gather_rows(gx[d].view(B * U, G4), src.view(-1), gxs)
                    hs = _new((U * B + 1, H), like=x, zero=True)
                    gx_s, h_s = (lambda t: gxs[t * B:(t + 1) * B]), (lambda t: hs[t * B:(t + 1) * B])
                gh = torch.empty(B, G4, dtype=torch.float32, device=x.device)
                for t in range(U):
                    if t > 0:
                        gemm_parts([stage_act_view(h_s(t - 1))], [whh], gh, block_n=64)
                    K.lstm_cell_fwd(gx_s(t), gh if t > 0 else None, cs[d][t - 1] if t > 0 else None, cs[d][t], h_s(t), gates[d][t], B, H)
                if not (lens is None and d == 0):
                    _, _, to_time = _lstm_step_maps(lens if lens is not None else _full_lens(B, U, x.device), B, U, d == 1)
                    ho = _new((B * U, H), like=x)
                    K.gather_rows(hs, to_time.t().contiguous().view(-1), ho)
                    out_d.copy_(ho.view(B, U, H))
        ctx.save_for_backward(x, out, gates, cs)
        ctx.x_parts, ctx.wih_parts, ctx.whh_parts = x_parts, wih_parts, whh_parts
        ctx.dirs, ctx.lens = dirs, lens
        return out

    @staticmethod
    def backward(ctx, dout):
        x, out, gates, cs = ctx.saved_tensors
        lens, dirs = ctx.lens, ctx.dirs
        n_dir = len(dirs)
        B, U, E = x.shape
        H = dirs[0][1].shape[1]
        G4 = 4 * H
        dout = dout.contiguous()
        dG = _new((n_dir, U, B, G4), like=out)
        if ctx.persistent:
            K.lstm_seq_bwd_ex(dout, gates, cs, ctx.whh_parts[0], dG, lens)
        else:
            dh_rec = torch.empty(B, H, dtype=torch.float32, device=x.device)
            dc = [torch.empty(B, H, dtype=torch.float32, device=x.device) for _ in range(2)]
            for d in range(n_dir):
                whh = [p[d * G4:(d + 1) * G4] for p in ctx.whh_parts]
                dout_d = dout[:, :, d * H:(d + 1) * H]
                if lens is None and d == 0:
                    do_s, dg_s = (lambda t: dout_d[:, t, :]), (lambda t: dG[d][t])
                else:
                    _, dsrc, to_time = _lstm_step_maps(lens if lens is not None else _full_lens(B, U, x.device), B, U, d == 1)
                    dz = torch.zeros(B * U + 1, H, dtype=dout.dtype, device=x.device)
                    dz[:B * U].view(B, U, H).copy_(dout_d)
                    dos = torch.empty(U * B, H, dtype=dout.dtype, device=x.device)
                    K.gather_rows(dz, dsrc.view(-1), dos)
                    dgs = _new((U * B + 1, G4), like=out, zero=True)
                    do_s, dg_s = (lambda t: dos[t * B:(t + 1) * B]), (lambda t: dgs[t * B:(t + 1) * B])
                for t in range(U - 1, -1, -1):
                    last = (t == U - 1)
                    K.lstm_cell_bwd(do_s(t), None if last else dh_rec, None if last else dc[(t + 1) & 1], gates[d][t], cs[d][t],
                                    cs[d][t - 1] if t > 0 else None, dg_s(t), dc[t & 1], B, H)
                    if t > 0:
                        gemm_parts([stage_act_view(dg_s(t))], [whh], dh_rec, b_mn=True, block_n=64)
                if not (lens is None and d == 0):
                    K.gather_rows(dgs, to_time.view(-1), dG[d].view(U * B, G4))
        dg_all = stage_act(dG)
        out_parts = stage_act(out)
        sel = dict(a_sel=(K.SEL_KZ, K.SEL_ZERO), b_sel=(K.SEL_KZ, K.SEL_ZERO))
        for d, (w_ih, w_hh, b_ih, b_hh) in enumerate(dirs):
            dg_parts = [p[d] for p in dg_all]
            h_parts = [p[:, :, d * H:(d + 1) * H].permute(1, 0, 2) for p in out_parts]
            if U > 1:
                a, b = ([p[1:] for p in dg_parts], [p[:-1] for p in h_parts]) if d == 0 else \
                       ([p[:-1] for p in dg_parts], [p[1:] for p in h_parts])
                gemm_parts([a], [b], grad_of(w_hh), a_mn=True, b_mn=True, kz_count=U - 1, **sel)
            else:
                grad_of(w_hh).zero_()
            gemm_parts([dg_parts], [[p.permute(1, 0, 2) for p in ctx.x_parts]], grad_of(w_ih), a_mn=True, b_mn=True, kz_count=U, **sel)
            K.colsum(dG[d].view(U * B, G4), grad_of(b_ih))
            grad_of(b_hh).copy_(b_ih.grad)
        dx = None
        if ctx.needs_input_grad[0]:
            dx = torch.empty_like(x)
            taps = [[p[d] for p in dg_all] for d in range(n_dir)]
            gemm_parts(taps, ctx.wih_parts, dx.permute(1, 0, 2), b_mn=True, a_sel=(K.SEL_ZB0, K.SEL_ZERO), b_sel=(K.SEL_ZERO, K.SEL_ZERO))
        return (dx, None) + (None,) * (4 * n_dir)


def _full_lens(B, U, device):
    return torch.full((B,), U, dtype=torch.int32, device=device)


def stage_act_view(v):
    if v.dtype == torch.bfloat16:
        return [v]
    hi = torch.empty(v.shape, dtype=torch.bfloat16, device=v.device)
    lo = torch.empty_like(hi)
    K.cast_split(v, hi, lo)
    return [hi, lo]


class DropoutFn(torch.autograd.Function):
    @staticmethod
    def forward(ctx, x, p, seed):
        y = torch.empty_like(x)
        K.dropout(x.contiguous(), y, p, seed)
        ctx.p, ctx.seed = p, seed
        return y

    @staticmethod
    def backward(ctx, dy):
        dx = torch.empty_like(dy)
        K.dropout(dy.contiguous(), dx, ctx.p, ctx.seed)
        return dx, None, None


def _ldv(V):
    return (V + 7) // 8 * 8


_FUSED_LSE = True


EVENT_TAPS = None


class _Tap:
    def __init__(self, name):
        self.name = name

    def __enter__(self):
        if EVENT_TAPS is not None:
            self.s = torch.cuda.Event(enable_timing=True)
            self.s.record()

    def __exit__(self, *exc):
        if EVENT_TAPS is not None:
            e = torch.cuda.Event(enable_timing=True)
            e.record()
            EVENT_TAPS.setdefault(self.name, []).append((self.s, e))


def _joint_forward(enc, pred, model, want_lse=False):
    B, T, H = enc.shape
    U1 = pred.shape[1]
    V = model.fc2.weight.shape[0]
    ldv = _ldv(V)
    fc1, fcg, fc2 = model.fc1, model.fc_gate, model.fc2
    wx = stage_weight([fc1.weight, fcg.weight])
    enc_parts = stage_act(enc.reshape(B * T, H))
    pred_parts = stage_act(pred.reshape(B * U1, H))
    ex = _new((B * T, 2 * H), like=enc)
    py = _new((B * U1, 2 * H), like=enc)
    gemm_parts([enc_parts], [[p[:, :H] for p in wx]], ex, bias=_cat_bias([fc1.bias, fcg.bias]))
    gemm_parts([pred_parts], [[p[:, H:] for p in wx]], py)
    R = B * T * U1
    h = _new((R, H), like=enc)
    K.joint_gate_fwd(ex, py, h, B, T, U1, H)
    w2 = stage_weight(fc2.weight)
    logits = _new((B, T, U1, ldv), like=enc, zero=(ldv != V))
    h_parts = stage_act(h)
    row_lse = None
    if want_lse and _FUSED_LSE and logits.dtype == torch.bfloat16 and V % 8 == 0:
        row_lse = torch.empty(K.row_lse_parts(R, V, 256), R, 2, dtype=torch.float32, device=enc.device)
    with _Tap("fc2_fwd"):
        gemm_parts([h_parts], [w2], logits.view(R, ldv)[:, :V], bias=fc2.bias.detach(), row_lse=row_lse,
                   **({"block_n": 256} if row_lse is not None else {}))
    state = dict(row_lse=row_lse, ex=ex, py=py, h_parts=h_parts, enc_parts=enc_parts, pred_parts=pred_parts, wx=wx, w2=w2, dims=(B, T, U1, H, V, ldv))
    return logits, state


def _joint_backward(dlogits, st, model, need_enc=True, need_pred=True, db2=None):
    B, T, U1, H, V, ldv = st["dims"]
    R = B * T * U1
    fc1, fcg, fc2 = model.fc1, model.fc_gate, model.fc2
    dl_parts = [p.view(R, ldv) for p in stage_act(dlogits)]
    dl_v = [p[:, :V] for p in dl_parts]
    dh = _new((R, H), like=dlogits)
    gemm_parts([dl_v], [st["w2"]], dh, b_mn=True)
    gemm_parts([dl_v], [st["h_parts"]], grad_of(fc2.weight), a_mn=True, b_mn=True)
    if db2 is None:
        db2 = torch.empty(ldv, dtype=torch.float32, device=dlogits.device)
        K.colsum(dlogits.view(R, ldv), db2)
    grad_of(fc2.bias).copy_(db2[:V])
    dex = _new((B * T, 2 * H), like=dlogits)
    dpy = _new((B * U1, 2 * H), like=dlogits)
    K.joint_gate_bwd(st["ex"], st["py"], dh, dex, dpy, B, T, U1, H)
    del dh
    dex_parts, dpy_parts = stage_act(dex), stage_act(dpy)
    g1, gg = grad_of(fc1.weight), grad_of(fcg.weight)
    for (dparts, xparts, lo) in ((dex_parts, st["enc_parts"], 0), (dpy_parts, st["pred_parts"], H)):
        gemm_parts([[p[:, :H] for p in dparts]], [xparts], g1[:, lo:lo + H], a_mn=True, b_mn=True)
        gemm_parts([[p[:, H:] for p in dparts]], [xparts], gg[:, lo:lo + H], a_mn=True, b_mn=True)
    dbx = torch.empty(2 * H, dtype=torch.float32, device=dlogits.device)
    K.colsum(dex, dbx)
    grad_of(fc1.bias).copy_(dbx[:H])
    grad_of(fcg.bias).copy_(dbx[H:])
    d_enc = d_pred = None
    if need_enc:
        d_enc = _new((B * T, H), like=dlogits)
        gemm_parts([dex_parts], [[p[:, :H] for p in st["wx"]]], d_enc, b_mn=True)
        d_enc = d_enc.view(B, T, H)
    if need_pred:
        d_pred = _new((B * U1, H), like=dlogits)
        gemm_parts([dpy_parts], [[p[:, H:] for p in st["wx"]]], d_pred, b_mn=True)
        d_pred = d_pred.view(B, U1, H)
    return d_enc, d_pred


class JointFn(torch.autograd.Function):

    @staticmethod
    def forward(ctx, enc, pred, model):
        logits, st = _joint_forward(enc, pred, model)
        ctx.st, ctx.model = st, model
        return logits

    @staticmethod
    def backward(ctx, dlogits):
        d_enc, d_pred = _joint_backward(dlogits.contiguous(), ctx.st, ctx.model, ctx.needs_input_grad[0], ctx.needs_input_grad[1])
        return d_enc, d_pred, None


_UNIT_LOSS_GRAD = False


def assume_unit_loss_grad(flag):
    global _UNIT_LOSS_GRAD
    _UNIT_LOSS_GRAD = bool(flag)


class JointLossFn(torch.autograd.Function):

    @staticmethod
    def forward(ctx, enc, pred, model, labels, frame_lens, label_lens, need_grad=True):
        logits, st = _joint_forward(enc, pred, model, want_lse=True)
        V = st["dims"][4]
        ctx.need_grad = need_grad
        if not need_grad:
            costs, _ = K.rnnt_loss_fwd_bwd(logits, labels, frame_lens, label_lens, V=V, want_grad=False, row_lse=st.pop("row_lse"))
            return costs
        db2 = torch.empty(logits.shape[-1], dtype=torch.float32, device=logits.device)
        with _Tap("rnnt_loss"):
            costs, _ = K.rnnt_loss_fwd_bwd(logits, labels, frame_lens, label_lens, V=V, dlogits=logits, colsum=db2,
                                           row_lse=st.pop("row_lse"))
        d_enc, d_pred = _joint_backward(logits, st, model, db2=db2)
        del logits, st
        ctx.save_for_backward(d_enc, d_pred)
        ctx.model = model
        return costs

    @staticmethod
    def backward(ctx, dcosts):
        if not ctx.need_grad:
            raise RuntimeError("JointLossFn: forward ran with grad mode off; there is nothing to back-propagate")
        d_enc, d_pred = ctx.saved_tensors
        if not _UNIT_LOSS_GRAD:
            w = dcosts.detach().float()
            if not bool((w == w[0]).all()):
                raise RuntimeError("JointLossFn: per-utterance loss weights are not supported by the fused joint backward "
                                   "(its parameter gradients were formed for a uniform upstream gradient)")
            if float(w[0]) != 1.0:
                m = ctx.model
                for p in (m.fc1.weight, m.fc1.bias, m.fc_gate.weight, m.fc_gate.bias, m.fc2.weight, m.fc2.bias):
                    p.grad.mul_(w[0])
                d_enc = d_enc * w[0].to(d_enc.dtype)
                d_pred = d_pred * w[0].to(d_pred.dtype)
        return d_enc, d_pred, None, None, None, None, None


class RNNTLossFn(torch.autograd.Function):

    @staticmethod
    def forward(ctx, log_probs, labels, frame_lens, label_lens):
        lp = log_probs.contiguous()
        B, T, U1, V = lp.shape
        ldv = V if (V % (8 if lp.dtype == torch.bfloat16 else 4) == 0) else None
        if ldv is None:
            ldv = _ldv(V)
            buf = torch.zeros(B, T, U1, ldv, dtype=lp.dtype, device=lp.device)
            buf[..., :V].copy_(lp)
            lp = buf
        costs, grads = K.rnnt_loss_fwd_bwd(lp, labels.int().contiguous(), frame_lens.int().contiguous(),
                                           label_lens.int().contiguous(), V=V)
        ctx.save_for_backward(grads[..., :V])
        return costs

    @staticmethod
    def backward(ctx, dcosts):
        (g,) = ctx.saved_tensors
        return g * dcosts.view(-1, 1, 1, 1).to(g.dtype), None, None, None


def _to_act(x):
    x = x.contiguous()
    if x.dtype == act_dtype():
        return x
    if act_dtype() == torch.bfloat16:
        x2 = x.reshape(-1, x.shape[-1]).float()
        out = torch.empty(x2.shape, dtype=torch.bfloat16, device=x.device)
        K.cast_split(x2, out)
        return out.view(x.shape)
    return x.float()


def transformer_layer(layer, x2, B, T, training, causal=False, key_pad=None):
    att, ff = layer.self_attn, layer.feed_forward
    p = _drop(layer.dropout_p, training)
    ln = LayerNormFn.apply(x2, layer.layer_norm, layer.layer_norm.weight, layer.layer_norm.bias)
    qkv = linear(ln, [att.linear_query.weight, att.linear_keys.weight, att.linear_values.weight],
                 [att.linear_query.bias, att.linear_keys.bias, att.linear_values.bias])
    rel = att.relative_positions_embeddings.weight if getattr(att, "max_relative_positions", 0) > 0 else None
    ctxv = AttentionFn.apply(qkv.view(B, T, -1), att.head_count, p, _next_seed() if p > 0 else 0, causal, key_pad, rel)
    h1 = linear(ctxv.view(B * T, -1), att.final_linear.weight, att.final_linear.bias, drop_p=p, residual=x2)
    ln2 = LayerNormFn.apply(h1, ff.layer_norm, ff.layer_norm.weight, ff.layer_norm.bias)
    fold = ln2.dtype == torch.bfloat16
    inter = linear(ln2, ff.w_1.weight, ff.w_1.bias, act=True, drop_p=p, premasked=fold)
    return linear(inter, ff.w_2.weight, ff.w_2.bias, drop_p=p, residual=h1,
                  mask_input_scale=(1.0 / (1.0 - p) if p > 0 else 1.0) if fold else 0.0)


def encoder_forward_act(enc, x, x_len=None, t_out=None):
    if isinstance(enc, torch.nn.LSTM):
        return lstm_encoder_forward_act(enc, x, x_len, t_out)
    training = enc.training
    B, T, D = x.shape
    C = enc.tdnn_nhid
    if T < 43:
        raise ValueError("encoder input has %d frames; the TDNN stack needs at least 43 (receptive field 21+1+21)" % T)
    h = linear(_to_act(x).view(B * T, D), enc.fc_in.weight, enc.fc_in.bias, act=True, premasked=True)
    h = BatchNormFn.apply(h, enc.bn_in, training, enc.bn_in.weight, enc.bn_in.bias, True)
    for l, (conv, bn) in enumerate(zip(enc.hidden_conv, enc.hidden_bn)):
        dil, stride = enc.TDNN_DIL_STRIDE[l]
        h3 = TdnnFn.apply(h.view(B, T, C), conv.weight, conv.bias, dil, stride, True)
        T = h3.shape[1]
        h = BatchNormFn.apply(h3.view(B * T, C), bn, training, bn.weight, bn.bias, True)
        if (l + 1) % 3 == 0:
            h = transformer_layer(enc.transformer[l // 3], h, B, T, training)
    h = BatchNormFn.apply(h, enc.bn_final, training, enc.bn_final.weight, enc.bn_final.bias)
    h = linear(h, enc.fc_out.weight, enc.fc_out.bias)
    return h.view(B, T, -1)


def encoder_forward(enc, x):
    return encoder_forward_act(enc, x).float()


def _lstm_layer_params(lstm, l):
    names = ["weight_ih_l%d", "weight_hh_l%d", "bias_ih_l%d", "bias_hh_l%d"]
    sfx = ["", "_reverse"] if lstm.bidirectional else [""]
    return [getattr(lstm, n % l + x) for x in sfx for n in names]


def lstm_encoder_forward_act(lstm, x, x_len=None, t_out=None):
    if lstm.batch_first is not True or not lstm.bias or lstm.proj_size:
        raise NotImplementedError("pika_b200: the LSTM encoder expects nn.LSTM(batch_first=True, bias=True, proj_size=0)")
    B, T, D = x.shape
    lens = None
    if x_len is None:
        t_out = T
    else:
        x_len = torch.as_tensor(x_len)
        if x_len.shape != (B,):
            raise ValueError("x_len must hold one length per sequence (%d), got shape %s" % (B, tuple(x_len.shape)))
        if t_out is None or not x_len.is_cuda:
            lo, hi = (int(v) for v in torch.stack((x_len.min(), x_len.max())).tolist())
            if lo < 1 or hi > T:
                raise ValueError("x_len must lie in [1, %d] (the frames of x); got [%d, %d]" % (T, lo, hi))
            t_out = hi if t_out is None else t_out
        if not 1 <= t_out <= T:
            raise ValueError("t_out = %d must lie in [1, %d]" % (t_out, T))
        lens = x_len.to(device=x.device, dtype=torch.int32).contiguous()
    ld = (D + 7) // 8 * 8
    h = _to_act(x[:, :t_out])
    if ld != D:
        hp = _new((B, t_out, ld), like=h, zero=True)
        hp[:, :, :D] = h
        h = hp
    p = _drop(lstm.dropout, lstm.training)
    for l in range(lstm.num_layers):
        h = LstmLayerFn.apply(h, lens, *_lstm_layer_params(lstm, l))
        if p > 0 and l < lstm.num_layers - 1:
            h = DropoutFn.apply(h, p, _next_seed())
    return h


def prednet_forward_act(model, y):
    B, U = y.shape
    sos = torch.zeros(B, 1, dtype=torch.long, device=y.device)
    yy = torch.cat((sos, y.long()), dim=1).contiguous()
    if getattr(model, "decoder_type", "rnn") != "rnn":
        return conv_transformer_lm_forward_act(model.decoder, yy)
    E = model.embed.weight.shape[1]
    ld = (E + 7) // 8 * 8
    h = EmbeddingFn.apply(yy, model.embed, ld, model.embed.weight).view(B, U + 1, ld)
    lstm = model.decoder
    p = _drop(lstm.dropout, lstm.training)
    for l in range(lstm.num_layers):
        h = LstmLayerFn.apply(h, None, *_lstm_layer_params(lstm, l))
        if p > 0 and l < lstm.num_layers - 1:
            h = DropoutFn.apply(h, p, _next_seed())
    return h


def conv_transformer_lm_forward_act(dec, src):
    B, L = src.shape
    emb = dec.embeddings
    ld = (emb.weight.shape[1] + 7) // 8 * 8
    src = src.contiguous()
    h = EmbeddingFn.apply(src, emb, ld, emb.weight).view(B, L, ld)
    key_pad = src.eq(emb.padding_idx).to(torch.uint8).contiguous() if emb.padding_idx is not None else None
    training = dec.training
    for conv, layer in zip(dec.conv, dec.transformer):
        assert conv.kernel_size[0] - 1 == conv.padding[0] and conv.dilation[0] == 1 and conv.stride[0] == 1
        h = CausalConvFn.apply(h, conv.weight, conv.bias)
        h = transformer_layer(layer, h.view(B * L, -1), B, L, training, causal=True, key_pad=key_pad).view(B, L, -1)
    hn = LayerNormFn.apply(h.reshape(B * L, -1), dec.layer_norm, dec.layer_norm.weight, dec.layer_norm.bias)
    return linear(hn, dec.linear_out.weight, dec.linear_out.bias).view(B, L, -1)


def model_encoder_forward_act(model, x, x_len=None, t_out=None):
    if getattr(model, "pack_seq", False):
        return encoder_forward_act(model.encoder, x, x_len, t_out)
    return encoder_forward_act(model.encoder, x)


def transducer_forward(model, x, y, softmax=True, x_len=None, t_out=None):
    enc = model_encoder_forward_act(model, x, x_len, t_out)
    pred = prednet_forward_act(model, y)
    logits = JointFn.apply(enc, pred, model)
    V = model.fc2.weight.shape[0]
    if not softmax:
        return logits[..., :V].float()
    return LogSoftmaxFn.apply(logits, V)


class LogSoftmaxFn(torch.autograd.Function):
    @staticmethod
    def forward(ctx, logits, V):
        out = torch.empty(logits.shape[:-1] + (V,), dtype=torch.float32, device=logits.device)
        K.log_softmax(logits, out, V)
        ctx.save_for_backward(out)
        ctx.ldv, ctx.dt = logits.shape[-1], logits.dtype
        return out

    @staticmethod
    def backward(ctx, dlp):
        (lp,) = ctx.saved_tensors
        g = dlp - lp.exp() * dlp.sum(-1, keepdim=True)
        out = torch.zeros(lp.shape[:-1] + (ctx.ldv,), dtype=ctx.dt, device=lp.device)
        out[..., :lp.shape[-1]] = g.to(ctx.dt)
        return out, None


def transducer_loss(model, x, y, frame_lens, label_lens, x_len=None, t_out=None):
    enc = model_encoder_forward_act(model, x, x_len, t_out)
    pred = prednet_forward_act(model, y)
    return JointLossFn.apply(enc, pred, model, y.int().contiguous(), frame_lens.int().contiguous(), label_lens.int().contiguous(),
                             torch.is_grad_enabled())
```

pika_b200/kernels.py:

```python
import ctypes

import torch

from . import _lib
from ._lib import (ACT_NONE, ACT_RELU, AUX_ADD, AUX_MASK_NZ, AUX_NONE, PK_BF16, PK_F32, SEL_KZ, SEL_ZB0, SEL_ZB1,
                   SEL_ZERO, GemmDesc, View4, check, lib)


def _stream():
    return ctypes.c_void_p(torch.cuda.current_stream().cuda_stream)


def _dt(t):
    if t.dtype == torch.bfloat16:
        return PK_BF16
    if t.dtype == torch.float32:
        return PK_F32
    raise TypeError("unsupported dtype %s" % t.dtype)


def _ptr(t):
    return ctypes.c_void_p(t.data_ptr()) if t is not None else ctypes.c_void_p(0)


def _fill_view(v, t):
    assert t.is_cuda and t.dim() >= 1 and t.dim() <= 4, "views must be CUDA tensors with 1..4 dims"
    assert t.stride(-1) == 1 or t.shape[-1] == 1, "innermost dimension must be contiguous"
    shape = list(t.shape)[::-1]
    strides = list(t.stride())[::-1]
    v.ptr = t.data_ptr()
    for i in range(4):
        v.dim[i] = shape[i] if i < len(shape) else 1
    for i in range(3):
        v.stride[i] = strides[i + 1] if i + 1 < len(strides) else 0
    return v


def gemm(a, b, c, a_mn=False, b_mn=False, a_sel=(SEL_ZB0, SEL_ZB1), b_sel=(SEL_ZB0, SEL_ZB1), kz_count=1,
         a_row_off=None, b_row_off=None, alpha=1.0, bias=None, act=ACT_NONE, drop_p=0.0, drop_seed=0,
         aux=None, aux_mode=AUX_NONE, aux_scale=1.0, accumulate=False, block_n=0, k_splits=0, row_lse=None):
    a = a if isinstance(a, (list, tuple)) else [a]
    b = b if isinstance(b, (list, tuple)) else [b]
    assert len(a) == len(b) and 1 <= len(a) <= _lib.MAX_PAIRS
    d = GemmDesc()
    d.n_pairs = len(a)
    for i, (ai, bi) in enumerate(zip(a, b)):
        assert ai.dtype == torch.bfloat16 and bi.dtype == torch.bfloat16, "GEMM operands must be bf16"
        _fill_view(d.a[i], ai)
        _fill_view(d.b[i], bi)
        d.a_row_off[i] = a_row_off[i] if a_row_off else 0
        d.b_row_off[i] = b_row_off[i] if b_row_off else 0
    d.a_mn_major, d.b_mn_major = int(a_mn), int(b_mn)
    d.a_sel2, d.a_sel3 = a_sel
    d.b_sel2, d.b_sel3 = b_sel
    d.kz_count = kz_count
    _fill_view(d.c, c)
    d.c_dtype = _dt(c)
    d.c_accumulate = int(accumulate)
    d.alpha = alpha
    if bias is not None:
        assert bias.dtype == torch.float32 and bias.is_contiguous()
        d.bias = bias.data_ptr()
    d.act = act
    d.drop_p = drop_p
    d.drop_seed = drop_seed & 0xFFFFFFFF
    if aux is not None:
        assert aux.dim() == c.dim() and aux.stride(-1) == 1
        d.aux_mode = aux_mode
        d.aux = aux.data_ptr()
        d.aux_dtype = _dt(aux)
        st = list(aux.stride())[::-1]
        for i in range(3):
            d.aux_stride[i] = st[i + 1] if i + 1 < len(st) else 0
        d.aux_scale = aux_scale
    d.block_n = block_n
    d.k_splits = k_splits
    if row_lse is not None:
        assert row_lse.dtype == torch.float32 and row_lse.is_contiguous() and c.dim() == 2
        assert tuple(row_lse.shape) == (row_lse_parts(c.shape[-2], c.shape[-1], block_n), c.shape[-2], 2)
        d.row_lse = row_lse.data_ptr()
    check(lib.pk_gemm_bf16(ctypes.byref(d), _stream()), "pk_gemm_bf16")
    return c


def row_lse_parts(M, N, block_n=0):
    return int(lib.pk_gemm_row_lse_parts(M, N, block_n))


def rnnt_loss_fwd_bwd(logits, labels, frame_lens, label_lens, V=None, grad_scale=None, dlogits=None, want_grad=True, colsum=None,
                      row_lse=None):
    B, T, U1, ldv = logits.shape
    V = ldv if V is None else V
    assert logits.is_contiguous() and labels.dtype == torch.int32 and labels.dim() == 2
    assert frame_lens.dtype == torch.int32 and label_lens.dtype == torch.int32
    ws_bytes = int(lib.pk_rnnt_loss_workspace_bytes(B, T, U1))
    if colsum is not None:
        ws_bytes += int(lib.pk_rnnt_loss_colsum_workspace_bytes(B, T, U1, ldv))
    ws = torch.empty(ws_bytes, dtype=torch.uint8, device=logits.device)
    costs = torch.empty(B, dtype=torch.float32, device=logits.device)
    if want_grad and dlogits is None:
        dlogits = torch.empty_like(logits)
    if row_lse is not None:
        assert row_lse.dtype == torch.float32 and row_lse.is_contiguous() and tuple(row_lse.shape[1:]) == (B * T * U1, 2)
        check(lib.pk_rnnt_loss_fwd_bwd_lse(_ptr(logits), _dt(logits), _ptr(labels), _ptr(frame_lens), _ptr(label_lens),
                                           B, T, U1, V, ldv, max(labels.stride(0), 1), _ptr(grad_scale), _ptr(costs),
                                           _ptr(dlogits if want_grad else None), _ptr(colsum), _ptr(ws), ws_bytes,
                                           _ptr(row_lse), int(row_lse.shape[0]), _stream()), "pk_rnnt_loss_fwd_bwd_lse")
        return costs, dlogits
    check(lib.pk_rnnt_loss_fwd_bwd(_ptr(logits), _dt(logits), _ptr(labels), _ptr(frame_lens), _ptr(label_lens),
                                   B, T, U1, V, ldv, max(labels.stride(0), 1), _ptr(grad_scale), _ptr(costs),
                                   _ptr(dlogits if want_grad else None), _ptr(colsum), _ptr(ws), ws_bytes, _stream()),
          "pk_rnnt_loss_fwd_bwd")
    return costs, dlogits


_P = lambda t: ctypes.c_void_p(t.data_ptr()) if t is not None else ctypes.c_void_p(0)
_L = ctypes.c_longlong
_I = ctypes.c_int
_F = ctypes.c_float
_U = ctypes.c_uint32


def cast_split(src, hi, lo=None, cols_pad=None, scale=1.0):
    rows, cols = src.shape
    cols_pad = cols_pad or cols
    assert hi.shape[-1] == cols_pad and hi.stride(-1) == 1 and src.stride(-1) == 1
    check(lib.pk_cast_split(_P(src), _I(_dt(src)), _L(src.stride(0)), _P(hi), _P(lo), _L(hi.stride(0)), _L(rows),
                            _I(cols), _I(cols_pad), _F(scale), _stream()), "pk_cast_split")


def attention_lse_stride(T):
    return int(lib.pk_attention_lse_stride(T))


def attention_fwd(qkv, out, lse, heads, alpha, drop_p=0.0, seed=0):
    B, T, D3 = qkv.shape
    D = D3 // 3
    assert qkv.dtype == torch.bfloat16 and qkv.is_contiguous() and out.is_contiguous() and out.shape == (B, T, D)
    assert lse.dtype == torch.float32 and lse.numel() == B * heads * attention_lse_stride(T)
    base, es = qkv.data_ptr(), 2
    vp = ctypes.c_void_p
    check(lib.pk_attention_fwd(vp(base), vp(base + D * es), vp(base + 2 * D * es), _L(D3), _P(out), _L(D), _P(lse), _I(B), _I(T),
                               _I(heads), _I(D // heads), _F(alpha), _F(drop_p), _U(seed & 0xFFFFFFFF), _stream()), "pk_attention_fwd")


def attention_bwd(qkv, out, dout, lse, dqkv, heads, alpha, drop_p=0.0, seed=0):
    B, T, D3 = qkv.shape
    D = D3 // 3
    assert dout.is_contiguous() and dqkv.is_contiguous() and dqkv.shape == qkv.shape and dout.dtype == torch.bfloat16
    ws = torch.zeros(B * heads * attention_lse_stride(T), dtype=torch.float32, device=qkv.device)
    base, gb, es = qkv.data_ptr(), dqkv.data_ptr(), 2
    vp = ctypes.c_void_p
    check(lib.pk_attention_bwd(vp(base), vp(base + D * es), vp(base + 2 * D * es), _L(D3), _P(out), _L(D), _P(dout), _L(D), _P(lse), _P(ws),
                               vp(gb), vp(gb + D * es), vp(gb + 2 * D * es), _L(D3), _I(B), _I(T), _I(heads), _I(D // heads), _F(alpha),
                               _F(drop_p), _U(seed & 0xFFFFFFFF), _stream()), "pk_attention_bwd")


_col_ws = {}


def col_ws(C, device):
    key = (C, str(device))
    if key not in _col_ws:
        lib.pk_colstats_ws_floats.restype = ctypes.c_longlong
        _col_ws[key] = torch.empty(int(lib.pk_colstats_ws_floats(C)) + 2 * C, dtype=torch.float32, device=device)
    return _col_ws[key]


def bn_fwd(x, y, w, b, eps, train, momentum, run_mean, run_var, mean, rstd, ws=None):
    rows, C = x.shape
    ws = col_ws(C, x.device)
    check(lib.pk_bn_fwd(_P(x), _P(y), _I(_dt(x)), _L(rows), _I(C), _P(w), _P(b), _F(eps), _I(int(train)), _F(momentum),
                        _P(run_mean), _P(run_var), _P(mean), _P(rstd), _P(ws), _stream()), "pk_bn_fwd")


def bn_bwd(dy, x, dx, w, mean, rstd, train, relu_mask, dw, db):
    rows, C = x.shape
    check(lib.pk_bn_bwd(_P(dy), _P(x), _P(dx), _I(_dt(x)), _L(rows), _I(C), _P(w), _P(mean), _P(rstd), _I(int(train)),
                        _I(int(relu_mask)), _P(dw), _P(db), _P(col_ws(C, x.device)), _stream()), "pk_bn_bwd")


def colsum(x, out):
    rows, C = x.shape
    assert x.is_contiguous()
    check(lib.pk_colsum(_P(x), _I(_dt(x)), _L(rows), _I(C), _P(out), _P(col_ws(C, x.device)), _stream()), "pk_colsum")


def layernorm_fwd(x, y, w, b, eps, mean, rstd):
    rows, C = x.shape
    check(lib.pk_layernorm_fwd(_P(x), _P(y), _I(_dt(x)), _L(rows), _I(C), _P(w), _P(b), _F(eps), _P(mean), _P(rstd),
                               _stream()), "pk_layernorm_fwd")


def layernorm_bwd(dy, x, dx, w, mean, rstd, dw, db):
    rows, C = x.shape
    check(lib.pk_layernorm_bwd(_P(dy), _P(x), _P(dx), _I(_dt(x)), _L(rows), _I(C), _P(w), _P(mean), _P(rstd), _P(dw),
                               _P(db), _stream()), "pk_layernorm_bwd")


def softmax_fwd(S, P, Pd, n, drop_p, seed):
    rows = S.numel() // S.shape[-1]
    check(lib.pk_softmax_fwd(_P(S), _L(S.shape[-1]), _P(P), _P(Pd), _I(_dt(P)), _L(P.shape[-1]), _L(rows), _I(n),
                             _F(drop_p), _U(seed & 0xFFFFFFFF), _stream()), "pk_softmax_fwd")


def softmax_masked_fwd(S, P, Pd, n, q_len, heads, causal, key_pad, drop_p, seed):
    rows = S.numel() // S.shape[-1]
    if key_pad is not None:
        assert key_pad.dtype == torch.uint8 and key_pad.is_contiguous() and key_pad.shape[-1] == n
    check(lib.pk_softmax_masked_fwd(_P(S), _L(S.shape[-1]), _P(P), _P(Pd), _I(_dt(P)), _L(P.shape[-1]), _L(rows), _I(n), _I(q_len),
                                    _I(heads), _I(int(bool(causal))), _P(key_pad), _F(drop_p), _U(seed & 0xFFFFFFFF), _stream()),
          "pk_softmax_masked_fwd")


def softmax_bwd(dPd, P, dS, n, drop_p, seed):
    rows = P.numel() // P.shape[-1]
    check(lib.pk_softmax_bwd(_P(dPd), _L(dPd.shape[-1]), _P(P), _L(P.shape[-1]), _P(dS), _I(_dt(P)), _L(rows), _I(n),
                             _F(drop_p), _U(seed & 0xFFFFFFFF), _stream()), "pk_softmax_bwd")


def softmax_masked_relpos_fwd(S, QR, P, Pd, Pb, n, heads, causal, key_pad, max_rel, drop_p, seed):
    rows = S.numel() // S.shape[-1]
    if key_pad is not None:
        assert key_pad.dtype == torch.uint8 and key_pad.is_contiguous() and key_pad.shape[-1] == n
    assert QR.dtype == torch.float32 and Pb.dtype == torch.float32 and QR.stride(-1) == 1 and Pb.stride() == QR.stride()
    check(lib.pk_softmax_masked_relpos_fwd(_P(S), _L(S.shape[-1]), _P(QR), _L(QR.stride(0)), _P(P), _P(Pd), _I(_dt(P)), _L(P.shape[-1]),
                                           _L(rows), _I(n), _I(n), _I(heads), _I(int(bool(causal))), _P(key_pad), _I(max_rel), _P(Pb),
                                           _F(drop_p), _U(seed & 0xFFFFFFFF), _stream()), "pk_softmax_masked_relpos_fwd")


def softmax_relpos_bwd(dPd, G, P, dS, dSb, n, heads, max_rel, drop_p, seed):
    rows = P.numel() // P.shape[-1]
    assert G.dtype == torch.float32 and dSb.dtype == torch.float32 and G.stride(-1) == 1 and dSb.stride() == G.stride()
    check(lib.pk_softmax_relpos_bwd(_P(dPd), _L(dPd.shape[-1]), _P(G), _L(G.stride(0)), _P(P), _L(P.shape[-1]), _P(dS), _I(_dt(P)),
                                    _L(rows), _I(n), _I(n), _I(heads), _I(max_rel), _P(dSb), _F(drop_p), _U(seed & 0xFFFFFFFF), _stream()),
          "pk_softmax_relpos_bwd")


def dropout(x, y, p, seed):
    check(lib.pk_dropout(_P(x), _P(y), _I(_dt(x)), _L(x.numel()), _F(p), _U(seed & 0xFFFFFFFF), _stream()), "pk_dropout")


def mask_nz(dy, y, dx, scale):
    check(lib.pk_mask_nz(_P(dy), _P(y), _P(dx), _I(_dt(y)), _L(y.numel()), _F(scale), _stream()), "pk_mask_nz")


def add(a, b, o):
    check(lib.pk_add(_P(a), _P(b), _P(o), _I(_dt(a)), _L(a.numel()), _stream()), "pk_add")


def log_softmax(x, y, n, scale=1.0):
    rows = x.numel() // x.shape[-1]
    check(lib.pk_log_softmax(_P(x), _I(_dt(x)), _L(x.shape[-1]), _P(y), _L(rows), _I(n), _F(scale), _stream()),
          "pk_log_softmax")


def joint_gate_fwd(ex, py, h, B, T, U1, H):
    check(lib.pk_joint_gate_fwd(_P(ex), _P(py), _P(h), _I(_dt(ex)), _I(B), _I(T), _I(U1), _I(H), _I(h.stride(0)), _stream()),
          "pk_joint_gate_fwd")


def joint_gate_bwd(ex, py, dh, dex, dpy, B, T, U1, H):
    check(lib.pk_joint_gate_bwd(_P(ex), _P(py), _P(dh), _P(dex), _P(dpy), _I(_dt(ex)), _I(B), _I(T), _I(U1), _I(H),
                                _stream()), "pk_joint_gate_bwd")


def lstm_cell_fwd(gx, gh, c_prev, c_out, h_out, gates_save, B, H):
    check(lib.pk_lstm_cell_fwd(_P(gx), _L(gx.stride(0)), _P(gh), _L(gh.stride(0) if gh is not None else 0), _P(c_prev),
                               _P(c_out), _P(h_out), _I(_dt(h_out)), _L(h_out.stride(0)), _P(gates_save), _I(B), _I(H),
                               _stream()), "pk_lstm_cell_fwd")


def lstm_cell_bwd(dh_out, dh_rec, dc_next, gates, c, c_prev, dgates, dc_prev, B, H):
    check(lib.pk_lstm_cell_bwd(_P(dh_out), _L(dh_out.stride(0) if dh_out is not None else 0), _P(dh_rec), _P(dc_next),
                               _P(gates), _P(c), _P(c_prev), _P(dgates), _I(_dt(dgates)), _P(dc_prev), _I(B), _I(H),
                               _stream()), "pk_lstm_cell_bwd")


def embedding_fwd(idx, table, out):
    n, ld = out.shape
    check(lib.pk_embedding_fwd(_P(idx), _P(table), _I(table.shape[1]), _P(out), _I(_dt(out)), _I(ld), _L(n), _stream()),
          "pk_embedding_fwd")


def embedding_bwd(idx, dout, dtable, padding_idx):
    n, ld = dout.shape
    check(lib.pk_embedding_bwd(_P(idx), _P(dout), _I(_dt(dout)), _I(ld), _I(dtable.shape[1]), _P(dtable), _L(n),
                               _L(padding_idx if padding_idx is not None else -1), _stream()), "pk_embedding_bwd")


def absmax(x, out, nan_flag=None):
    check(lib.pk_absmax(_P(x), _L(x.numel()), _P(out), _P(nan_flag), _stream()), "pk_absmax")


def sgd_nesterov_clip(p, g, buf, lr, momentum, max_norm, absmax_t, first, nan_flag=None):
    check(lib.pk_sgd_nesterov_clip(_P(p), _P(g), _P(buf), _L(p.numel()), _F(lr), _F(momentum), _F(max_norm), _P(absmax_t),
                                   _P(nan_flag), _I(int(first)), _stream()), "pk_sgd_nesterov_clip")


def bmuf_delta(glob, local, delta):
    check(lib.pk_bmuf_delta(_P(glob), _P(local), _P(delta), _L(glob.numel()), _stream()), "pk_bmuf_delta")


def bmuf_update(glob, local, delta_prev, delta_sum, world, bm, blr):
    check(lib.pk_bmuf_update(_P(glob), _P(local), _P(delta_prev), _P(delta_sum), _L(glob.numel()), _I(world), _F(bm), _F(blr),
                             _stream()), "pk_bmuf_update")


_lstm_ws = {}


def _lstm_scratch(H, device):
    key = (H, str(device))
    if key not in _lstm_ws:
        lib.pk_lstm_seq_workspace_bytes.restype = ctypes.c_longlong
        _lstm_ws[key] = torch.zeros(int(lib.pk_lstm_seq_workspace_bytes(H)), dtype=torch.uint8, device=device)
    return _lstm_ws[key]


def _lens_arg(lens, B):
    if lens is None:
        return ctypes.c_void_p(0)
    assert lens.dtype == torch.int32 and lens.is_contiguous() and lens.numel() == B
    return _P(lens)


def lstm_seq_fwd_ex(gx, w_hh, out, gates_save, cs, lens=None, reverse=False):
    n_dir, B, U, G4 = gx.shape
    H = G4 // 4
    assert gx.is_contiguous() and w_hh.dtype == torch.bfloat16 and w_hh.is_contiguous() and w_hh.shape[0] == n_dir * G4
    assert out.stride(2) == 1 and out.stride(0) == U * out.stride(1) and out.shape[-1] == n_dir * H
    check(lib.pk_lstm_seq_fwd_ex(_P(gx), _P(w_hh), _P(out), _I(_dt(out)), _I(out.stride(1)), _P(gates_save), _P(cs), _lens_arg(lens, B),
                                 _I(B), _I(U), _I(H), _I(n_dir), _I(int(reverse)), _P(_lstm_scratch(n_dir * H, gx.device)), _stream()),
          "pk_lstm_seq_fwd_ex")


def lstm_seq_bwd_ex(dout, gates_save, cs, w_hh, dG, lens=None, reverse=False):
    n_dir, U, B, G4 = dG.shape
    H = G4 // 4
    assert dout.stride(2) == 1 and dout.stride(0) == U * dout.stride(1) and dout.shape[-1] == n_dir * H
    assert dG.dtype == torch.bfloat16 and dG.is_contiguous() and w_hh.shape[0] == n_dir * G4
    check(lib.pk_lstm_seq_bwd_ex(_P(dout), _I(_dt(dout)), _I(dout.stride(1)), _P(gates_save), _P(cs), _P(w_hh), _P(dG), _lens_arg(lens, B),
                                 _I(B), _I(U), _I(H), _I(n_dir), _I(int(reverse)), _P(_lstm_scratch(n_dir * H, dout.device)), _stream()),
          "pk_lstm_seq_bwd_ex")


def gather_rows(src, idx, dst):
    rows, C = dst.shape
    check(lib.pk_gather_rows(_P(src), _P(idx), _P(dst), _I(_dt(src)), _L(rows), _I(C), _stream()), "pk_gather_rows")


def scatter_add_rows(src, idx, dst):
    rows, C = src.shape
    assert dst.dtype == torch.float32
    check(lib.pk_scatter_add_rows(_P(src), _P(idx), _P(dst), _I(_dt(src)), _L(rows), _I(C), _stream()), "pk_scatter_add_rows")


class BeamXfState(ctypes.Structure):
    _fields_ = [("next_ys", ctypes.c_void_p), ("step_ctx", ctypes.c_void_p), ("hyp_tok", ctypes.c_void_p), ("hyp_len", ctypes.c_void_p),
                ("slot", ctypes.c_void_p), ("pool", ctypes.c_void_p), ("n_entries", ctypes.c_longlong), ("blk", ctypes.c_int),
                ("rows", ctypes.c_int), ("S1", ctypes.c_int), ("layers", ctypes.c_int), ("D", ctypes.c_int), ("dtype", ctypes.c_int),
                ("init", ctypes.c_int)]


def beam_xf_taps(st, layer, embed, x_cur, taps):
    assert embed.dtype == torch.float32 and embed.is_contiguous() and taps.is_contiguous()
    check(lib.pk_beam_xf_taps(ctypes.byref(st), _I(layer), _P(embed), _I(embed.shape[1]), _P(x_cur), _P(taps), _I(taps.shape[1] // 5),
                              _stream()), "pk_beam_xf_taps")


def beam_xf_attn(st, layer, qkv, heads, rel, out):
    assert qkv.is_contiguous() and out.is_contiguous() and (rel is None or (rel.dtype == torch.float32 and rel.is_contiguous()))
    check(lib.pk_beam_xf_attn(ctypes.byref(st), _I(layer), _P(qkv), _I(heads), _P(rel), _I(0 if rel is None else rel.shape[0] // 2), _P(out),
                              _stream()), "pk_beam_xf_attn")


def beam_xf_select(st, x, h):
    check(lib.pk_beam_xf_select(ctypes.byref(st), _P(x), _P(h), _I(h.shape[-1]), _stream()), "pk_beam_xf_select")


def beam_xf_slots(st, prev_ks, K):
    check(lib.pk_beam_xf_slots(ctypes.byref(st), _P(prev_ks), _I(K), _stream()), "pk_beam_xf_slots")


def ce_grad(z, tok, coef, scale, dz, n):
    rows, ld = z.shape
    check(lib.pk_ce_grad(_P(z), _I(_dt(z)), _L(ld), _P(tok), _P(coef), _F(scale), _P(dz), _L(rows), _I(n), _stream()), "pk_ce_grad")
```

Measured before the change: 264.6.

## Store attention dropout keep-mask as bits in forward, reuse in backward

The fused attention forward now writes the dropout keep decisions as packed bitmasks to a global buffer. Both backward passes read that buffer instead of recomputing the hash-based dropout mask; the dK/dV pass streams it through the TMA ring into shared memory. This removes repeated per-element hash evaluations in backward, especially the costly transposed salt recomputation in mode 2. In exchange it adds global memory writes and reads of the mask and extra shared memory. The forward loop is also restructured to hoist fragment packing and apply the rescale after the softmax.

```diff
diff --git a/include/pika_b200.h b/include/pika_b200.h
--- a/include/pika_b200.h
+++ b/include/pika_b200.h
@@ -74,11 +74,18 @@
 int pk_cast_split(const void* src, int src_dtype, long long ld_src, void* hi, void* lo, long long ld_dst,
                   long long rows, int cols, int cols_pad, float scale, void* stream);
 int pk_attention_lse_stride(int T);
+long long pk_attention_keep_bits_bytes(int B, int T, int heads);
 int pk_attention_fwd(const void* q, const void* k, const void* v, long long ld_qkv, void* out, long long ld_out, float* lse,
                      int B, int T, int heads, int dh, float alpha, float drop_p, uint32_t seed, void* stream);
 int pk_attention_bwd(const void* q, const void* k, const void* v, long long ld_qkv, const void* out, long long ld_out,
                      const void* dout, long long ld_dout, const float* lse, float* dsum_ws, void* dq, void* dk, void* dv,
                      long long ld_dqkv, int B, int T, int heads, int dh, float alpha, float drop_p, uint32_t seed, void* stream);
+int pk_attention_fwd_bits(const void* q, const void* k, const void* v, long long ld_qkv, void* out, long long ld_out, float* lse,
+                          int B, int T, int heads, int dh, float alpha, float drop_p, uint32_t seed, uint32_t* keep_bits, void* stream);
+int pk_attention_bwd_bits(const void* q, const void* k, const void* v, long long ld_qkv, const void* out, long long ld_out,
+                          const void* dout, long long ld_dout, const float* lse, float* dsum_ws, void* dq, void* dk, void* dv,
+                          long long ld_dqkv, int B, int T, int heads, int dh, float alpha, float drop_p, const uint32_t* keep_bits,
+                          void* stream);
 long long pk_colstats_ws_floats(int C);
 int pk_bn_fwd(const void* x, void* y, int dtype, long long rows, int C, const float* w, const float* b, float eps,
               int train, float momentum, float* run_mean, float* run_var, float* mean, float* rstd, float* stats_ws,
diff --git a/pika_b200/_lib.py b/pika_b200/_lib.py
--- a/pika_b200/_lib.py
+++ b/pika_b200/_lib.py
@@ -71,6 +71,7 @@
 _sig("pk_gemm_bf16", [ctypes.POINTER(GemmDesc), _vp])
 _sig("pk_gemm_row_lse_parts", [_ll, _ll, _i])
 _sig("pk_rnnt_loss_workspace_bytes", [_i, _i, _i], ctypes.c_longlong)
+_sig("pk_attention_keep_bits_bytes", [_i, _i, _i], ctypes.c_longlong)
 _sig("pk_rnnt_loss_colsum_workspace_bytes", [_i, _i, _i, _i], ctypes.c_longlong)
 _sig("pk_rnnt_loss_fwd_bwd", [_vp, _i, _vp, _vp, _vp, _i, _i, _i, _i, _i, _i, _vp, _vp, _vp, _vp, _vp, _ll, _vp])
 _sig("pk_rnnt_loss_fwd_bwd_lse", [_vp, _i, _vp, _vp, _vp, _i, _i, _i, _i, _i, _i, _vp, _vp, _vp, _vp, _vp, _ll, _vp, _i, _vp])
diff --git a/pika_b200/csrc/attention_tc.cu b/pika_b200/csrc/attention_tc.cu
--- a/pika_b200/csrc/attention_tc.cu
+++ b/pika_b200/csrc/attention_tc.cu
@@ -19,7 +19,10 @@
 constexpr int TA_OFF_STAT = 0;
 constexpr int TA_OFF_RING = 2 * TA_TILE_S;
 constexpr int TA_OFF_VEC = TA_OFF_RING + TA_NST * 2 * TA_TILE_X;
-constexpr int TA_OFF_BAR = TA_OFF_VEC + TA_NST * 2 * TA_BC * 4;
+enum : int { TA_DROP_NONE = 0, TA_DROP_HASH = 1, TA_DROP_BITS = 2 };
+constexpr int TA_KB_BLOCK = 512;
+constexpr int TA_OFF_KB = TA_OFF_VEC + TA_NST * 2 * TA_BC * 4;
+constexpr int TA_OFF_BAR = TA_OFF_KB + TA_NST * 2 * TA_KB_BLOCK;
 constexpr int TA_SMEM = TA_OFF_BAR + 256 + 1024;
 
 struct AttnTcParams {
@@ -28,7 +31,8 @@
     __nv_bfloat16* dq; __nv_bfloat16* dk; __nv_bfloat16* dv; long long ld_dqkv;
     float* lse;
     float* dsum;
-    int B, T, heads, Tpad, Tp2;
+    uint32_t* keep_bits;
+    int B, T, heads, Tpad, Tp2, nkb;
     float alpha;
     uint32_t thresh16; float drop_scale; uint32_t seed;
 };
@@ -39,6 +43,7 @@
     a[2] = pack_bf16x2(x[8 * kk + 4], x[8 * kk + 5]);
     a[3] = pack_bf16x2(x[8 * kk + 6], x[8 * kk + 7]);
 }
+PK_DEVICE size_t kb_block(const AttnTcParams& p, int bh, int qb, int kb) { return (((size_t)bh * p.nkb + qb) * p.nkb + kb) * (TA_KB_BLOCK / 4); }
 PK_DEVICE float quad_max(float v) { return fmaxf(v, fmaxf(__shfl_xor_sync(0xffffffffu, v, 1), __shfl_xor_sync(0xffffffffu, fmaxf(v, __shfl_xor_sync(0xffffffffu, v, 1)), 2))); }
 PK_DEVICE float quad_sum(float v) { v += __shfl_xor_sync(0xffffffffu, v, 1); return v + __shfl_xor_sync(0xffffffffu, v, 2); }
 
@@ -54,7 +59,7 @@
     }
 }
 
-template <int MODE>
+template <int MODE, int DROP>
 __global__ void __launch_bounds__(TA_THREADS, 1) attention_tc_kernel(const __grid_constant__ AttnTcParams p) {
     extern __shared__ uint8_t smem_raw[];
     uint8_t* smem = reinterpret_cast<uint8_t*>((reinterpret_cast<uintptr_t>(smem_raw) + 1023) & ~uintptr_t(1023));
@@ -92,18 +97,22 @@
             tma_load_3d_p(smem + TA_OFF_STAT + half * TA_TILE_X, ma0, stat_full, h * 64, row_base + half * 64, b, lead);
             if (MODE != 0) tma_load_3d_p(smem + TA_OFF_STAT + TA_TILE_S + half * TA_TILE_X, ma1, stat_full, h * 64, row_base + half * 64, b, lead);
         }
+        constexpr bool kb_load = MODE == 2 && DROP == TA_DROP_BITS;
         int stage = 0;
         uint32_t phase = 0;
         for (int j = 0; j < n_tiles; ++j) {
             mbar_wait(&empty_bar[stage], phase ^ 1);
             uint8_t* x1 = smem + TA_OFF_RING + stage * 2 * TA_TILE_X;
-            mbar_arrive_expect_tx_p(&full_bar[stage], 2 * TA_TILE_X + (MODE == 2 ? 2 * TA_BC * 4 : 0), lead);
+            mbar_arrive_expect_tx_p(&full_bar[stage], 2 * TA_TILE_X + (MODE == 2 ? 2 * TA_BC * 4 : 0) + (kb_load ? 2 * TA_KB_BLOCK : 0), lead);
             tma_load_3d_p(x1, mx1, &full_bar[stage], h * 64, j * TA_BC, b, lead);
             tma_load_3d_p(x1 + TA_TILE_X, mx2, &full_bar[stage], h * 64, j * TA_BC, b, lead);
             if (MODE == 2) {
                 const size_t off = (size_t)bh * p.Tpad + (size_t)j * TA_BC;
                 bulk_load_p(vec + (stage * 2 + 0) * TA_BC, p.lse + off, TA_BC * 4, &full_bar[stage], lead);
                 bulk_load_p(vec + (stage * 2 + 1) * TA_BC, p.dsum + off, TA_BC * 4, &full_bar[stage], lead);
+                if (kb_load)
+                    bulk_load_p(smem + TA_OFF_KB + stage * 2 * TA_KB_BLOCK, p.keep_bits + kb_block(p, bh, j, 2 * blockIdx.x), 2 * TA_KB_BLOCK,
+                                &full_bar[stage], lead);
             }
             if (++stage == TA_NST) { stage = 0; phase ^= 1; }
         }
@@ -118,19 +127,20 @@
     const int srow0 = row_base + wg * 64;
     const uint64_t stat_row0 = (uint64_t)bh * (uint64_t)T;
     const float c2 = p.alpha * TA_LOG2E;
-    const bool use_drop = p.thresh16 != 0u;
+    constexpr bool use_drop = DROP != TA_DROP_NONE, KB = DROP == TA_DROP_BITS;
     const uint32_t sbase = smem_u32(smem);
     const uint64_t kdesc = make_smem_desc_sw128(0, 16, 1024);
     const uint64_t mdesc = make_smem_desc_sw128(0, 8192, 1024);
     auto kmaj = [&](uint32_t addr, int k4) { return kdesc + (uint64_t)((addr >> 4) & 0x3FFF) + (uint64_t)(k4 * 2); };
     auto mnmaj = [&](uint32_t addr, int k4) { return mdesc + (uint64_t)((addr >> 4) & 0x3FFF) + (uint64_t)(k4 * 128); };
     const uint32_t st0 = sbase + TA_OFF_STAT + wg * TA_TILE_X, st1 = st0 + TA_TILE_S;
+    const int kb_word = (et >> 5) * 32 + (lane & 3) * 8 + (lane >> 2);
     uint32_t row_salt[2];
     float lse2[2] = {0.f, 0.f}, dsum_r[2] = {0.f, 0.f};
 #pragma unroll
     for (int hh = 0; hh < 2; ++hh) {
         const int srow = srow0 + r0 + 8 * hh;
-        row_salt[hh] = drop_row_salt(stat_row0 + (uint64_t)srow, p.seed);
+        if (MODE == 0 || (MODE == 1 && !KB)) row_salt[hh] = drop_row_salt(stat_row0 + (uint64_t)srow, p.seed);
         if (MODE == 1 && srow < T) {
             lse2[hh] = p.lse[(size_t)bh * p.Tpad + srow] * TA_LOG2E;
             dsum_r[hh] = p.dsum[(size_t)bh * p.Tpad + srow];
@@ -143,41 +153,35 @@
     float m_run[2] = {-INFINITY, -INFINITY}, l_run[2] = {0.f, 0.f};
 
     mbar_wait(stat_full, 0);
-    int stage = 0;
-    uint32_t phase = 0;
-    for (int j = 0; j < n_tiles; ++j) {
-        const int col0 = j * TA_BC;
-        const int nvalid = min(TA_BC, T - col0);
-        mbar_wait(&full_bar[stage], phase);
-        const uint32_t x1 = sbase + TA_OFF_RING + stage * 2 * TA_TILE_X, x2 = x1 + TA_TILE_X;
-        float s[32], dp[32];
-        wgmma_fence_acc(s);
-        wgmma_fence();
-#pragma unroll
-        for (int k4 = 0; k4 < 4; ++k4) wgmma_ss_n64<0, 0>(s, kmaj(st0, k4), kmaj(x1, k4), k4 > 0 ? 1u : 0u);
-        if (MODE != 0) {
-            wgmma_fence_acc(dp);
-#pragma unroll
-            for (int k4 = 0; k4 < 4; ++k4) wgmma_ss_n64<0, 0>(dp, kmaj(st1, k4), kmaj(x2, k4), k4 > 0 ? 1u : 0u);
-        }
-        wgmma_commit();
-        wgmma_wait<0>();
-        wgmma_fence_acc(s);
-        if (MODE != 0) wgmma_fence_acc(dp);
-        if (nvalid < TA_BC) {
-#pragma unroll
-            for (int c = 0; c < 32; ++c) if ((c >> 2) * 8 + cq + (c & 1) >= nvalid) s[c] = -INFINITY;
-        }
-        if (MODE == 0) {
+    if (MODE == 0) {
+        int stage = 0;
+        uint32_t phase = 0;
+        for (int j = 0; j < n_tiles; ++j) {
+            const int col0 = j * TA_BC;
+            const int nvalid = min(TA_BC, T - col0);
+            mbar_wait(&full_bar[stage], phase);
+            const uint32_t x1 = sbase + TA_OFF_RING + stage * 2 * TA_TILE_X, x2 = x1 + TA_TILE_X;
+            float s[32];
+            wgmma_fence_acc(s);
+            wgmma_fence();
+#pragma unroll
+            for (int k4 = 0; k4 < 4; ++k4) wgmma_ss_n64<0, 0>(s, kmaj(st0, k4), kmaj(x1, k4), k4 > 0 ? 1u : 0u);
+            wgmma_commit();
+            wgmma_wait<0>();
+            wgmma_fence_acc(s);
+            if (nvalid < TA_BC) {
+#pragma unroll
+                for (int c = 0; c < 32; ++c) if ((c >> 2) * 8 + cq + (c & 1) >= nvalid) s[c] = -INFINITY;
+            }
+            uint32_t kbits = 0u;
+            float corr[2];
 #pragma unroll
             for (int hh = 0; hh < 2; ++hh) {
                 float mx = -INFINITY;
 #pragma unroll
                 for (int nb = 0; nb < 8; ++nb) mx = fmaxf(mx, fmaxf(s[nb * 4 + 2 * hh], s[nb * 4 + 2 * hh + 1]));
                 const float m_new = fmaxf(m_run[hh], quad_max(mx) * c2);
-                const float corr = ex2_approx(m_run[hh] - m_new);
-#pragma unroll
-                for (int nb = 0; nb < 8; ++nb) { acc0[nb * 4 + 2 * hh] *= corr; acc0[nb * 4 + 2 * hh + 1] *= corr; }
+                corr[hh] = ex2_approx(m_run[hh] - m_new);
                 float sum = 0.f;
 #pragma unroll
                 for (int nb = 0; nb < 8; ++nb) {
@@ -189,79 +193,123 @@
                         const uint32_t km = drop_pair(row_salt[hh], (uint32_t)((col0 + nb * 8 + cq) >> 1), p.thresh16);
                         if (!(km & 1u)) pr[0] = 0.f;
                         if (!(km & 2u)) pr[1] = 0.f;
+                        kbits |= km << (hh * 16 + nb * 2);
                     }
                 }
-                l_run[hh] = l_run[hh] * corr + sum;
+                l_run[hh] = l_run[hh] * corr[hh] + sum;
                 m_run[hh] = m_new;
             }
+            if (KB) __stcs(p.keep_bits + kb_block(p, bh, 2 * blockIdx.x + wg, j) + kb_word, kbits);
+            uint32_t a[4][4];
+#pragma unroll
+            for (int kk = 0; kk < 4; ++kk) frag_a(s, kk, a[kk]);
+#pragma unroll
+            for (int c = 0; c < 32; ++c) acc0[c] *= corr[(c >> 1) & 1];
             wgmma_fence_acc(acc0);
             wgmma_fence();
 #pragma unroll
-            for (int kk = 0; kk < 4; ++kk) {
-                uint32_t a[4];
-                frag_a(s, kk, a);
-                wgmma_rs_n64<1>(acc0, a, mnmaj(x2, kk), 1u);
-            }
-        } else {
-            float pd[32], ds[32];
-            const float* lse_t = vec + (stage * 2 + 0) * TA_BC;
-            const float* dsum_t = lse_t + TA_BC;
-            uint32_t qsalt[16];
-            if (MODE == 2 && use_drop) {
-#pragma unroll
-                for (int c = 0; c < 16; ++c) qsalt[c] = drop_row_salt(stat_row0 + (uint64_t)(col0 + (c >> 1) * 8 + cq + (c & 1)), p.seed);
-            }
-#pragma unroll
-            for (int hh = 0; hh < 2; ++hh) {
-#pragma unroll
-                for (int nb = 0; nb < 8; ++nb) {
-                    uint32_t keep = 3u;
-                    if (use_drop) {
-                        if (MODE == 1) {
-                            keep = drop_pair(row_salt[hh], (uint32_t)((col0 + nb * 8 + cq) >> 1), p.thresh16);
-                        } else {
-                            const uint32_t key = (uint32_t)(srow0 + r0 + 8 * hh);
-                            const uint32_t bit = (key & 1u) ? 2u : 1u;
-                            keep = ((drop_pair(qsalt[2 * nb], key >> 1, p.thresh16) & bit) ? 1u : 0u) |
-                                   ((drop_pair(qsalt[2 * nb + 1], key >> 1, p.thresh16) & bit) ? 2u : 0u);
+            for (int kk = 0; kk < 4; ++kk) wgmma_rs_n64<1>(acc0, a[kk], mnmaj(x2, kk), 1u);
+            wgmma_commit();
+            wgmma_wait<0>();
+            wgmma_fence_acc(acc0);
+            if (et == 0) mbar_arrive(&empty_bar[stage]);
+            if (++stage == TA_NST) { stage = 0; phase ^= 1; }
+        }
+    } else {
+        int stage = 0;
+        uint32_t phase = 0;
+        for (int j = 0; j < n_tiles; ++j) {
+            const int col0 = j * TA_BC;
+            uint32_t kw = 0u;
+            if (MODE == 1 && KB && use_drop) kw = __ldg(p.keep_bits + kb_block(p, bh, 2 * blockIdx.x + wg, j) + kb_word);
+            mbar_wait(&full_bar[stage], phase);
+            const uint32_t x1 = sbase + TA_OFF_RING + stage * 2 * TA_TILE_X, x2 = x1 + TA_TILE_X;
+            float s[32], dp[32];
+            wgmma_fence_acc(s);
+            wgmma_fence();
+#pragma unroll
+            for (int k4 = 0; k4 < 4; ++k4) wgmma_ss_n64<0, 0>(s, kmaj(st0, k4), kmaj(x1, k4), k4 > 0 ? 1u : 0u);
+            wgmma_fence_acc(dp);
+#pragma unroll
+            for (int k4 = 0; k4 < 4; ++k4) wgmma_ss_n64<0, 0>(dp, kmaj(st1, k4), kmaj(x2, k4), k4 > 0 ? 1u : 0u);
+            wgmma_commit();
+            wgmma_wait<0>();
+            wgmma_fence_acc(s);
+            wgmma_fence_acc(dp);
+            {
+                float pd[32], ds[32];
+                const float* lse_t = vec + (stage * 2 + 0) * TA_BC;
+                const float* dsum_t = lse_t + TA_BC;
+                uint32_t kq[4][2], qsalt[16];
+                if (MODE == 2 && !KB && use_drop) {
+#pragma unroll
+                    for (int c = 0; c < 16; ++c) qsalt[c] = drop_row_salt(stat_row0 + (uint64_t)(col0 + (c >> 1) * 8 + cq + (c & 1)), p.seed);
+                }
+                if (MODE == 2 && KB && use_drop) {
+                    const uint32_t kb_addr = sbase + TA_OFF_KB + (stage * 2 + wg) * TA_KB_BLOCK + ((lane >> 3) * 8 + cq) * 4;
+                    const int sh = (et >> 5) * 4 + ((lane >> 2) & 1);
+#pragma unroll
+                    for (int m = 0; m < 4; ++m) {
+                        const uint2 v = lds_u32x2(kb_addr + m * 128);
+                        kq[m][0] = v.x >> sh;
+                        kq[m][1] = v.y >> sh;
+                    }
+                }
+#pragma unroll
+                for (int hh = 0; hh < 2; ++hh) {
+#pragma unroll
+                    for (int nb = 0; nb < 8; ++nb) {
+                        uint32_t keep = 3u;
+                        if (use_drop) {
+                            if (MODE == 1) {
+                                keep = KB ? (kw >> (hh * 16 + nb * 2)) & 3u
+                                          : drop_pair(row_salt[hh], (uint32_t)((col0 + nb * 8 + cq) >> 1), p.thresh16);
+                            } else if (KB) {
+                                const int bit = (nb & 1) * 16 + 2 * hh;
+                                keep = ((kq[nb >> 1][0] >> bit) & 1u) | (((kq[nb >> 1][1] >> bit) & 1u) << 1);
+                            } else {
+                                const uint32_t key = (uint32_t)(srow0 + r0 + 8 * hh);
+                                const uint32_t bit = (key & 1u) ? 2u : 1u;
+                                keep = ((drop_pair(qsalt[2 * nb], key >> 1, p.thresh16) & bit) ? 1u : 0u) |
+                                       ((drop_pair(qsalt[2 * nb + 1], key >> 1, p.thresh16) & bit) ? 2u : 0u);
+                            }
+                        }
+#pragma unroll
+                        for (int e = 0; e < 2; ++e) {
+                            const int c = nb * 4 + 2 * hh + e;
+                            const int cl = nb * 8 + cq + e;
+                            const float l2 = (MODE == 1) ? lse2[hh] : lse_t[cl] * TA_LOG2E;
+                            const float dd = (MODE == 1) ? dsum_r[hh] : dsum_t[cl];
+                            const float pr = ex2_approx(fmaf(s[c], c2, -l2));
+                            const bool kp = (keep >> e) & 1u;
+                            const float dpe = kp ? dp[c] * p.drop_scale : 0.f;
+                            ds[c] = pr * (dpe - dd);
+                            if (MODE == 2) pd[c] = kp ? pr * p.drop_scale : 0.f;
                         }
                     }
-#pragma unroll
-                    for (int e = 0; e < 2; ++e) {
-                        const int c = nb * 4 + 2 * hh + e;
-                        const int cl = nb * 8 + cq + e;
-                        const float l2 = (MODE == 1) ? lse2[hh] : lse_t[cl] * TA_LOG2E;
-                        const float dd = (MODE == 1) ? dsum_r[hh] : dsum_t[cl];
-                        const float pr = ex2_approx(fmaf(s[c], c2, -l2));
-                        const bool kp = (keep >> e) & 1u;
-                        const float dpe = kp ? dp[c] * p.drop_scale : 0.f;
-                        ds[c] = pr * (dpe - dd);
-                        if (MODE == 2) pd[c] = kp ? pr * p.drop_scale : 0.f;
-                    }
+                }
+                uint32_t a[4][4], a2[4][4];
+#pragma unroll
+                for (int kk = 0; kk < 4; ++kk) {
+                    frag_a(ds, kk, a[kk]);
+                    if (MODE == 2) frag_a(pd, kk, a2[kk]);
+                }
+                wgmma_fence_acc(acc0);
+                if (MODE == 2) wgmma_fence_acc(acc1);
+                wgmma_fence();
+#pragma unroll
+                for (int kk = 0; kk < 4; ++kk) {
+                    wgmma_rs_n64<1>(acc0, a[kk], mnmaj(x1, kk), 1u);
+                    if (MODE == 2) wgmma_rs_n64<1>(acc1, a2[kk], mnmaj(x2, kk), 1u);
                 }
             }
+            wgmma_commit();
+            wgmma_wait<0>();
             wgmma_fence_acc(acc0);
             if (MODE == 2) wgmma_fence_acc(acc1);
-            wgmma_fence();
-#pragma unroll
-            for (int kk = 0; kk < 4; ++kk) {
-                uint32_t a[4];
-                frag_a(ds, kk, a);
-                if (MODE == 1) wgmma_rs_n64<1>(acc0, a, mnmaj(x1, kk), 1u);
-                else wgmma_rs_n64<1>(acc0, a, mnmaj(x1, kk), 1u);
-                if (MODE == 2) {
-                    uint32_t a2[4];
-                    frag_a(pd, kk, a2);
-                    wgmma_rs_n64<1>(acc1, a2, mnmaj(x2, kk), 1u);
-                }
-            }
-        }
-        wgmma_commit();
-        wgmma_wait<0>();
-        wgmma_fence_acc(acc0);
-        if (MODE == 2) wgmma_fence_acc(acc1);
-        if (et == 0) mbar_arrive(&empty_bar[stage]);
-        if (++stage == TA_NST) { stage = 0; phase ^= 1; }
+            if (et == 0) mbar_arrive(&empty_bar[stage]);
+            if (++stage == TA_NST) { stage = 0; phase ^= 1; }
+        }
     }
 
     if (MODE == 0) {
@@ -319,8 +367,8 @@
     return 0;
 }
 
-template <int MODE> static int launch_attn(const AttnTcParams& p, cudaStream_t st) {
-    auto kern = attention_tc_kernel<MODE>;
+template <int MODE, int DROP> static int launch_attn_drop(const AttnTcParams& p, cudaStream_t st) {
+    auto kern = attention_tc_kernel<MODE, DROP>;
     static bool configured = false;
     if (!configured) {
         PK_CHECK_CUDA(cudaFuncSetAttribute(kern, cudaFuncAttributeMaxDynamicSharedMemorySize, TA_SMEM));
@@ -331,12 +379,21 @@
     PK_CHECK_LAUNCH(); count_launch();
     return 0;
 }
+template <int MODE> static int launch_attn(const AttnTcParams& p, cudaStream_t st) {
+    if (p.thresh16 == 0u) return launch_attn_drop<MODE, TA_DROP_NONE>(p, st);
+    return p.keep_bits ? launch_attn_drop<MODE, TA_DROP_BITS>(p, st) : launch_attn_drop<MODE, TA_DROP_HASH>(p, st);
+}
 
 }
 
 #define STREAM(s) reinterpret_cast<cudaStream_t>(s)
 
 extern "C" int pk_attention_lse_stride(int T) { return (T + 63) / 64 * 64; }
+static int attn_kb_blocks(int T) { return (T + 127) / 128 * 2; }
+extern "C" long long pk_attention_keep_bits_bytes(int B, int T, int heads) {
+    const long long n = attn_kb_blocks(T);
+    return (long long)B * heads * n * n * pk::TA_KB_BLOCK;
+}
 
 #define ATTN_CHECKS()                                                                                                      \
     PK_CHECK_ARG(B > 0 && T > 0 && heads > 0, "bad dims");                                                                 \
@@ -344,14 +401,18 @@
     PK_CHECK_ARG(ld_qkv % 8 == 0 && ld_out % 8 == 0, "row strides must be multiples of 8 elements (16 bytes)");            \
     PK_CHECK_ARG(drop_p >= 0.f && drop_p < 1.f, "drop_p out of range");                                                    \
     PK_CHECK_ARG((long long)B * heads < 65536, "B * heads must be < 65536")
-
-extern "C" int pk_attention_fwd(const void* q, const void* k, const void* v, long long ld_qkv, void* out, long long ld_out, float* lse,
-                                int B, int T, int heads, int dh, float alpha, float drop_p, uint32_t seed, void* stream) {
+#define KEEP_BITS_CHECK()                                                                                                  \
+    PK_CHECK_ARG(drop_p == 0.f || (keep_bits != nullptr && ((uintptr_t)keep_bits & 15) == 0),                               \
+                 "keep_bits must be a 16-byte aligned buffer of pk_attention_keep_bits_bytes when drop_p > 0")
+
+static int attention_fwd(const void* q, const void* k, const void* v, long long ld_qkv, void* out, long long ld_out, float* lse,
+                         int B, int T, int heads, int dh, float alpha, float drop_p, uint32_t seed, uint32_t* keep_bits, void* stream) {
     using namespace pk;
     ATTN_CHECKS();
     static thread_local AttnTcParams p;
     memset(&p, 0, sizeof(p));
     p.B = B; p.T = T; p.heads = heads; p.Tpad = pk_attention_lse_stride(T); p.Tp2 = (T + 1) / 2;
+    p.keep_bits = drop_p > 0.f ? keep_bits : nullptr; p.nkb = attn_kb_blocks(T);
     int rc = attn_maps(p, q, k, v, ld_qkv, nullptr, 0);
     if (rc) return rc;
     p.out = (__nv_bfloat16*)out; p.ld_o = ld_out; p.lse = lse;
@@ -360,15 +421,17 @@
     return launch_attn<0>(p, STREAM(stream));
 }
 
-extern "C" int pk_attention_bwd(const void* q, const void* k, const void* v, long long ld_qkv, const void* out, long long ld_out,
-                                const void* dout, long long ld_dout, const float* lse, float* dsum_ws, void* dq, void* dk, void* dv,
-                                long long ld_dqkv, int B, int T, int heads, int dh, float alpha, float drop_p, uint32_t seed, void* stream) {
+static int attention_bwd(const void* q, const void* k, const void* v, long long ld_qkv, const void* out, long long ld_out,
+                         const void* dout, long long ld_dout, const float* lse, float* dsum_ws, void* dq, void* dk, void* dv,
+                         long long ld_dqkv, int B, int T, int heads, int dh, float alpha, float drop_p, uint32_t seed,
+                         const uint32_t* keep_bits, void* stream) {
     using namespace pk;
     ATTN_CHECKS();
     PK_CHECK_ARG(ld_dout % 8 == 0 && ld_dqkv % 8 == 0, "row strides must be multiples of 8 elements (16 bytes)");
     static thread_local AttnTcParams p;
     memset(&p, 0, sizeof(p));
     p.B = B; p.T = T; p.heads = heads; p.Tpad = pk_attention_lse_stride(T); p.Tp2 = (T + 1) / 2;
+    p.keep_bits = drop_p > 0.f ? const_cast<uint32_t*>(keep_bits) : nullptr; p.nkb = attn_kb_blocks(T);
     int rc = attn_maps(p, q, k, v, ld_qkv, dout, ld_dout);
     if (rc) return rc;
     p.dq = (__nv_bfloat16*)dq; p.dk = (__nv_bfloat16*)dk; p.dv = (__nv_bfloat16*)dv; p.ld_dqkv = ld_dqkv;
@@ -385,3 +448,28 @@
     if (rc) return rc;
     return launch_attn<2>(p, STREAM(stream));
 }
+
+extern "C" int pk_attention_fwd(const void* q, const void* k, const void* v, long long ld_qkv, void* out, long long ld_out, float* lse,
+                                int B, int T, int heads, int dh, float alpha, float drop_p, uint32_t seed, void* stream) {
+    return attention_fwd(q, k, v, ld_qkv, out, ld_out, lse, B, T, heads, dh, alpha, drop_p, seed, nullptr, stream);
+}
+extern "C" int pk_attention_fwd_bits(const void* q, const void* k, const void* v, long long ld_qkv, void* out, long long ld_out, float* lse,
+                                     int B, int T, int heads, int dh, float alpha, float drop_p, uint32_t seed, uint32_t* keep_bits,
+                                     void* stream) {
+    KEEP_BITS_CHECK();
+    return attention_fwd(q, k, v, ld_qkv, out, ld_out, lse, B, T, heads, dh, alpha, drop_p, seed, keep_bits, stream);
+}
+extern "C" int pk_attention_bwd(const void* q, const void* k, const void* v, long long ld_qkv, const void* out, long long ld_out,
+                                const void* dout, long long ld_dout, const float* lse, float* dsum_ws, void* dq, void* dk, void* dv,
+                                long long ld_dqkv, int B, int T, int heads, int dh, float alpha, float drop_p, uint32_t seed, void* stream) {
+    return attention_bwd(q, k, v, ld_qkv, out, ld_out, dout, ld_dout, lse, dsum_ws, dq, dk, dv, ld_dqkv, B, T, heads, dh, alpha, drop_p, seed,
+                         nullptr, stream);
+}
+extern "C" int pk_attention_bwd_bits(const void* q, const void* k, const void* v, long long ld_qkv, const void* out, long long ld_out,
+                                     const void* dout, long long ld_dout, const float* lse, float* dsum_ws, void* dq, void* dk, void* dv,
+                                     long long ld_dqkv, int B, int T, int heads, int dh, float alpha, float drop_p, const uint32_t* keep_bits,
+                                     void* stream) {
+    KEEP_BITS_CHECK();
+    return attention_bwd(q, k, v, ld_qkv, out, ld_out, dout, ld_dout, lse, dsum_ws, dq, dk, dv, ld_dqkv, B, T, heads, dh, alpha, drop_p, 0u,
+                         keep_bits, stream);
+}
diff --git a/pika_b200/csrc/common.cuh b/pika_b200/csrc/common.cuh
--- a/pika_b200/csrc/common.cuh
+++ b/pika_b200/csrc/common.cuh
@@ -310,6 +310,11 @@
     asm volatile("ld.shared.v4.u32 {%0, %1, %2, %3}, [%4];" : "=r"(v.x), "=r"(v.y), "=r"(v.z), "=r"(v.w) : "r"(addr) : "memory");
     return v;
 }
+PK_DEVICE uint2 lds_u32x2(uint32_t addr) {
+    uint2 v;
+    asm volatile("ld.shared.v2.u32 {%0, %1}, [%2];" : "=r"(v.x), "=r"(v.y) : "r"(addr) : "memory");
+    return v;
+}
 PK_DEVICE float2 lds_f32x2(uint32_t addr) {
     float2 v;
     asm volatile("ld.shared.v2.f32 {%0, %1}, [%2];" : "=f"(v.x), "=f"(v.y) : "r"(addr) : "memory");
diff --git a/pika_b200/csrc/runtime.cu b/pika_b200/csrc/runtime.cu
--- a/pika_b200/csrc/runtime.cu
+++ b/pika_b200/csrc/runtime.cu
@@ -29,5 +29,5 @@
 }
 
 extern "C" const char* pk_last_error(void) { return pk::g_err; }
-extern "C" int pk_version(void) { return 102; }
+extern "C" int pk_version(void) { return 103; }
 extern "C" long long pk_launch_count(void) { return pk::g_launches.load(); }
diff --git a/pika_b200/engine.py b/pika_b200/engine.py
--- a/pika_b200/engine.py
+++ b/pika_b200/engine.py
@@ -398,8 +398,9 @@
             out = _new((B, T, D), like=qkv)
             lse = torch.zeros(B * heads * K.attention_lse_stride(T), dtype=torch.float32, device=qkv.device)
             alpha = 1.0 / math.sqrt(dh)
-            K.attention_fwd(qkv, out, lse, heads, alpha, drop_p, seed)
-            ctx.save_for_backward(qkv, out, lse)
+            keep_bits = K.attention_keep_bits(B, T, heads, drop_p, qkv.device)
+            K.attention_fwd(qkv, out, lse, heads, alpha, drop_p, seed, keep_bits=keep_bits)
+            ctx.save_for_backward(qkv, out, lse, keep_bits)
             ctx.meta = (B, T, D, heads, dh, 0, drop_p, seed, alpha)
             return out
         Tp = (T + 7) // 8 * 8
@@ -447,10 +448,10 @@
     @staticmethod
     def backward(ctx, dout):
         if ctx.fused:
-            qkv, out, lse = ctx.saved_tensors
+            qkv, out, lse, keep_bits = ctx.saved_tensors
             B, T, D, heads, dh, _, drop_p, seed, alpha = ctx.meta
             dqkv = torch.empty_like(qkv)
-            K.attention_bwd(qkv, out, dout.contiguous(), lse, dqkv, heads, alpha, drop_p, seed)
+            K.attention_bwd(qkv, out, dout.contiguous(), lse, dqkv, heads, alpha, drop_p, seed, keep_bits=keep_bits)
             return dqkv, None, None, None, None, None, None
         qkv, P = ctx.saved_tensors
         B, T, D, heads, dh, Tp, drop_p, seed, alpha = ctx.meta
diff --git a/pika_b200/kernels.py b/pika_b200/kernels.py
--- a/pika_b200/kernels.py
+++ b/pika_b200/kernels.py
@@ -133,27 +133,41 @@
     return int(lib.pk_attention_lse_stride(T))
 
 
-def attention_fwd(qkv, out, lse, heads, alpha, drop_p=0.0, seed=0):
+def attention_keep_bits(B, T, heads, drop_p, device):
+    if drop_p <= 0:
+        return None
+    return torch.empty(int(lib.pk_attention_keep_bits_bytes(B, T, heads)) // 4, dtype=torch.int32, device=device)
+
+
+def attention_fwd(qkv, out, lse, heads, alpha, drop_p=0.0, seed=0, keep_bits=None):
     B, T, D3 = qkv.shape
     D = D3 // 3
     assert qkv.dtype == torch.bfloat16 and qkv.is_contiguous() and out.is_contiguous() and out.shape == (B, T, D)
     assert lse.dtype == torch.float32 and lse.numel() == B * heads * attention_lse_stride(T)
     base, es = qkv.data_ptr(), 2
     vp = ctypes.c_void_p
-    check(lib.pk_attention_fwd(vp(base), vp(base + D * es), vp(base + 2 * D * es), _L(D3), _P(out), _L(D), _P(lse), _I(B), _I(T),
-                               _I(heads), _I(D // heads), _F(alpha), _F(drop_p), _U(seed & 0xFFFFFFFF), _stream()), "pk_attention_fwd")
-
-
-def attention_bwd(qkv, out, dout, lse, dqkv, heads, alpha, drop_p=0.0, seed=0):
+    args = (vp(base), vp(base + D * es), vp(base + 2 * D * es), _L(D3), _P(out), _L(D), _P(lse), _I(B), _I(T), _I(heads), _I(D // heads),
+            _F(alpha), _F(drop_p), _U(seed & 0xFFFFFFFF))
+    if keep_bits is None:
+        check(lib.pk_attention_fwd(*args, _stream()), "pk_attention_fwd")
+        return
+    assert keep_bits.is_contiguous() and keep_bits.numel() * keep_bits.element_size() >= lib.pk_attention_keep_bits_bytes(B, T, heads)
+    check(lib.pk_attention_fwd_bits(*args, _P(keep_bits), _stream()), "pk_attention_fwd_bits")
+
+
+def attention_bwd(qkv, out, dout, lse, dqkv, heads, alpha, drop_p=0.0, seed=0, keep_bits=None):
     B, T, D3 = qkv.shape
     D = D3 // 3
     assert dout.is_contiguous() and dqkv.is_contiguous() and dqkv.shape == qkv.shape and dout.dtype == torch.bfloat16
     ws = torch.zeros(B * heads * attention_lse_stride(T), dtype=torch.float32, device=qkv.device)
     base, gb, es = qkv.data_ptr(), dqkv.data_ptr(), 2
     vp = ctypes.c_void_p
-    check(lib.pk_attention_bwd(vp(base), vp(base + D * es), vp(base + 2 * D * es), _L(D3), _P(out), _L(D), _P(dout), _L(D), _P(lse), _P(ws),
-                               vp(gb), vp(gb + D * es), vp(gb + 2 * D * es), _L(D3), _I(B), _I(T), _I(heads), _I(D // heads), _F(alpha),
-                               _F(drop_p), _U(seed & 0xFFFFFFFF), _stream()), "pk_attention_bwd")
+    args = (vp(base), vp(base + D * es), vp(base + 2 * D * es), _L(D3), _P(out), _L(D), _P(dout), _L(D), _P(lse), _P(ws),
+            vp(gb), vp(gb + D * es), vp(gb + 2 * D * es), _L(D3), _I(B), _I(T), _I(heads), _I(D // heads), _F(alpha), _F(drop_p))
+    if keep_bits is None:
+        check(lib.pk_attention_bwd(*args, _U(seed & 0xFFFFFFFF), _stream()), "pk_attention_bwd")
+    else:
+        check(lib.pk_attention_bwd_bits(*args, _P(keep_bits), _stream()), "pk_attention_bwd_bits")
 
 
 _col_ws = {}
```

Result: faster. 275.7 (median of 6 runs) (+4.2%).
